# bacchus-snu/bacchus-gpu-controller

Measured on AMD Instinct MI355X. Metric: reconcile p99 (ms) + admission p50 (ms); CR apply→Ready/sec on 8×MI355X node, higher is better.
Workload: dtype none

## Files before the change

native/apiserver/fieldset.cc:

```cpp
#include "apiserver/fieldset.h"

#include "core/json_patch.h"

namespace bgc::apiserver {

using json::Value;

namespace {

enum class ListKind { Atomic, KeyedByUid, Set };

ListKind list_kind(const std::string& path) {
  if (path == "/metadata/ownerReferences") return ListKind::KeyedByUid;
  if (path == "/metadata/finalizers") return ListKind::Set;
  return ListKind::Atomic;
}

bool ignored(const std::string& path, bool include_status) {
  static const std::set<std::string> kIgnored = {
      "/apiVersion", "/kind", "/metadata/name", "/metadata/namespace", "/metadata/resourceVersion",
      "/metadata/uid", "/metadata/generation", "/metadata/creationTimestamp", "/metadata/managedFields",
      "/metadata/selfLink", "/metadata/deletionTimestamp", "/metadata/deletionGracePeriodSeconds"};
  if (kIgnored.count(path)) return true;
  if (!include_status && (path == "/status" || path.rfind("/status/", 0) == 0)) return true;
  return false;
}

void collect(const Value& v, const std::string& path, FieldSet& out, bool include_status) {
  if (!path.empty() && ignored(path, include_status)) return;
  if (v.is_object() && !v.empty()) {
    const auto& keys = v.keys();
    const auto& vals = v.values();
    for (size_t i = 0; i < keys.size(); ++i) {
      collect(vals[i], path + "/" + json::escape_pointer_token(keys[i]), out, include_status);
    }
    return;
  }
  if (v.is_array() && !v.empty()) {
    ListKind lk = list_kind(path);
    if (lk == ListKind::KeyedByUid) {
      for (const auto& item : v.items()) {
        out.insert(path + "/[uid=" + json::escape_pointer_token(item.get_string("uid")) + "]");
      }
      return;
    }
    if (lk == ListKind::Set) {
      for (const auto& item : v.items()) out.insert(path + "/[=" + json::escape_pointer_token(item.dump()) + "]");
      return;
    }
  }
  if (!path.empty()) out.insert(path);
}

class Tokens {
 public:
  explicit Tokens(std::string_view p) : p_(p), i_(p.empty() ? 1 : 1), end_(p.empty()) {}
  bool next(std::string_view& tok) {
    if (end_ || i_ > p_.size()) return false;
    size_t j = p_.find('/', i_);
    std::string_view raw = p_.substr(i_, j == std::string_view::npos ? std::string_view::npos : j - i_);
    if (j == std::string_view::npos) end_ = true;
    else i_ = j + 1;
    if (raw.find('~') == std::string_view::npos) {
      tok = raw;
      return true;
    }
    scratch_.clear();
    for (size_t k = 0; k < raw.size(); ++k) {
      if (raw[k] == '~' && k + 1 < raw.size()) {
        scratch_.push_back(raw[k + 1] == '1' ? '/' : '~');
        ++k;
      } else {
        scratch_.push_back(raw[k]);
      }
    }
    tok = scratch_;
    return true;
  }
  bool last() const { return end_; }

 private:
  std::string_view p_;
  size_t i_;
  bool end_;
  std::string scratch_;
};

bool is_item_token(std::string_view t) { return t.size() >= 3 && t.front() == '[' && t.back() == ']'; }

long find_item(const Value& arr, std::string_view tok) {
  std::string_view inner = tok.substr(1, tok.size() - 2);
  if (inner.substr(0, 4) == "uid=") {
    std::string_view uid = inner.substr(4);
    for (size_t i = 0; i < arr.size(); ++i) {
      const Value& u = arr[i].get("uid");
      if (u.is_string() && u.as_string() == uid) return static_cast<long>(i);
    }
    return -1;
  }
  if (!inner.empty() && inner.front() == '=') {
    Value want;
    if (!json::try_parse(inner.substr(1), want, nullptr)) return -1;
    for (size_t i = 0; i < arr.size(); ++i) {
      if (arr[i] == want) return static_cast<long>(i);
    }
  }
  return -1;
}

}

FieldSet leaves(const Value& obj, bool include_status) {
  FieldSet fs;
  collect(obj, "", fs, include_status);
  return fs;
}

const Value* get_path(const Value& root, const std::string& path) {
  const Value* cur = &root;
  Tokens ts(path);
  std::string_view t;
  while (ts.next(t)) {
    if (is_item_token(t)) {
      if (!cur->is_array()) return nullptr;
      long i = find_item(*cur, t);
      if (i < 0) return nullptr;
      cur = &(*cur)[static_cast<size_t>(i)];
    } else {
      cur = cur->find(t);
      if (!cur) return nullptr;
    }
  }
  return cur;
}

bool remove_path(Value& root, const std::string& path) {
  Value* cur = &root;
  Tokens ts(path);
  std::string_view t;
  while (ts.next(t)) {
    const bool last = ts.last();
    if (is_item_token(t)) {
      if (!cur->is_array()) return false;
      long i = find_item(*cur, t);
      if (i < 0) return false;
      if (last) {
        cur->erase_index(static_cast<size_t>(i));
        return true;
      }
      cur = &(*cur)[static_cast<size_t>(i)];
    } else {
      if (last) return cur->erase(t);
      cur = cur->find_mut(t);
      if (!cur) return false;
    }
  }
  return false;
}

void set_path(Value& root, const std::string& path, const Value& v) {
  Value* cur = &root;
  Tokens ts(path);
  std::string_view t;
  while (ts.next(t)) {
    const bool last = ts.last();
    if (is_item_token(t)) {
      if (!cur->is_array()) *cur = Value::array();
      long i = find_item(*cur, t);
      if (i < 0) {
        cur->push_back(last ? v : Value::object());
        cur = &(*cur)[cur->size() - 1];
      } else {
        cur = &(*cur)[static_cast<size_t>(i)];
        if (last) *cur = v;
      }
      continue;
    }
    if (!cur->is_object()) *cur = Value::object();
    if (last) {
      (*cur)[t] = v;
    } else {
      cur = &(*cur)[t];
    }
  }
}

void diff_leaves(const Value& before, const Value& after, FieldSet& changed, FieldSet& removed, bool include_status) {
  FieldSet b = leaves(before, include_status);
  FieldSet a = leaves(after, include_status);
  for (const auto& p : a) {
    const Value* bv = b.count(p) ? get_path(before, p) : nullptr;
    const Value* av = get_path(after, p);
    if (!bv || !av || !(*bv == *av)) changed.insert(p);
  }
  for (const auto& p : b) {
    if (!a.count(p)) removed.insert(p);
  }
}

void diff_member_leaves(const Value& before, const Value& after, const std::string& key, FieldSet& changed,
                        FieldSet& removed) {
  const std::string base = "/" + json::escape_pointer_token(key);
  FieldSet b, a;
  if (const Value* v = before.find(key)) collect(*v, base, b, true);
  if (const Value* v = after.find(key)) collect(*v, base, a, true);
  for (const auto& p : a) {
    const Value* bv = b.count(p) ? get_path(before, p) : nullptr;
    const Value* av = get_path(after, p);
    if (!bv || !av || !(*bv == *av)) changed.insert(p);
  }
  for (const auto& p : b) {
    if (!a.count(p)) removed.insert(p);
  }
}

std::string display_path(const std::string& path) {
  std::string out;
  Tokens ts(path);
  std::string_view t;
  while (ts.next(t)) {
    if (!is_item_token(t)) out += '.';
    out.append(t.data(), t.size());
  }
  return out;
}

Value fields_v1(const FieldSet& fs) {
  Value root = Value::object();
  for (const auto& p : fs) {
    Value* cur = &root;
    Tokens ts(p);
    std::string_view t;
    std::string key;
    while (ts.next(t)) {
      key.clear();
      if (is_item_token(t)) {
        std::string_view inner = t.substr(1, t.size() - 2);
        if (inner.substr(0, 4) == "uid=") key = "k:{\"uid\":" + json::quote(std::string(inner.substr(4))) + "}";
        else key.append("v:").append(inner.substr(1));
      } else {
        key.append("f:").append(t);
      }
      cur = &(*cur)[key];
      if (cur->is_null()) *cur = Value::object();
    }
  }
  return root;
}

}
```

native/apiserver/fieldset.h:

```cpp
#pragma once

#include <map>
#include <set>
#include <string>
#include <vector>

#include "core/json.h"

namespace bgc::apiserver {

using FieldSet = std::set<std::string>;

FieldSet leaves(const json::Value& obj, bool include_status = false);
const json::Value* get_path(const json::Value& root, const std::string& path);
bool remove_path(json::Value& root, const std::string& path);
void set_path(json::Value& root, const std::string& path, const json::Value& v);
void diff_leaves(const json::Value& before, const json::Value& after, FieldSet& changed, FieldSet& removed,
                 bool include_status = false);
void diff_member_leaves(const json::Value& before, const json::Value& after, const std::string& key,
                        FieldSet& changed, FieldSet& removed);
std::string display_path(const std::string& path);
json::Value fields_v1(const FieldSet& fs);

}
```

native/apiserver/server.cc:

```cpp
#include "apiserver/server.h"

#include <algorithm>
#include <array>
#include <atomic>
#include <chrono>
#include <condition_variable>
#include <deque>
#include <functional>
#include <iterator>
#include <mutex>
#include <optional>
#include <regex>
#include <set>
#include <sstream>
#include <thread>
#include <unordered_map>
#include <unordered_set>

#include <openssl/crypto.h>

#include "apiserver/fieldset.h"
#include "core/crypto.h"
#include "core/http.h"
#include "core/json_patch.h"
#include "core/log.h"
#include "core/metrics.h"
#include "core/process.h"
#include "core/stall.h"
#include "core/trace.h"
#include "core/net.h"
#include "core/yaml.h"
#include "crd/schema.h"
#include "kube/leader.h"
#include "kube/quantity.h"
#include "kube/resource.h"

namespace bgc::apiserver {

using json::Value;
using kube::ResourceType;

namespace {


struct StatusError : std::runtime_error {
  int code;
  std::string reason;
  Value details;
  StatusError(int c, std::string r, const std::string& msg, Value d = {})
      : std::runtime_error(msg), code(c), reason(std::move(r)), details(std::move(d)) {}
};

Value status_body(int code, const std::string& reason, const std::string& message, const Value& details = {}) {
  Value s = Value::object({{"kind", "Status"}, {"apiVersion", "v1"}, {"metadata", Value::object()},
                           {"status", code < 400 ? "Success" : "Failure"}, {"message", message},
                           {"reason", reason}});
  if (!details.is_null()) s["details"] = details;
  s["code"] = code;
  return s;
}

std::string resource_ref(const ResourceType& rt) {
  return rt.group.empty() ? rt.plural : rt.plural + "." + rt.group;
}

StatusError not_found(const ResourceType& rt, const std::string& name) {
  return StatusError(404, "NotFound", resource_ref(rt) + " \"" + name + "\" not found",
                     Value::object({{"name", name}, {"group", rt.group}, {"kind", rt.plural}}));
}

StatusError already_exists(const ResourceType& rt, const std::string& name) {
  return StatusError(409, "AlreadyExists", resource_ref(rt) + " \"" + name + "\" already exists",
                     Value::object({{"name", name}, {"group", rt.group}, {"kind", rt.plural}}));
}

StatusError conflict(const ResourceType& rt, const std::string& name) {
  return StatusError(409, "Conflict",
                     "Operation cannot be fulfilled on " + resource_ref(rt) + " \"" + name +
                         "\": the object has been modified; please apply your changes to the latest version and try again",
                     Value::object({{"name", name}, {"group", rt.group}, {"kind", rt.plural}}));
}

StatusError invalid(const ResourceType& rt, const std::string& name, const std::string& msg) {
  return StatusError(422, "Invalid", rt.kind + "." + rt.group + " \"" + name + "\" is invalid: " + msg,
                     Value::object({{"name", name}, {"group", rt.group}, {"kind", rt.kind}}));
}

std::string now_rfc3339() {
  std::string s = kube::rfc3339_micro_now();
  return s.substr(0, 19) + "Z";
}

bool dns1123_label(const std::string& s) {
  if (s.empty() || s.size() > 63) return false;
  for (size_t i = 0; i < s.size(); ++i) {
    char c = s[i];
    bool ok = (c >= 'a' && c <= 'z') || (c >= '0' && c <= '9') || (c == '-' && i != 0 && i + 1 != s.size());
    if (!ok) return false;
  }
  return true;
}

bool dns1123_subdomain(const std::string& s) {
  if (s.empty() || s.size() > 253) return false;
  size_t start = 0;
  while (true) {
    size_t dot = s.find('.', start);
    std::string part = s.substr(start, dot == std::string::npos ? std::string::npos : dot - start);
    if (!dns1123_label(part)) return false;
    if (dot == std::string::npos) return true;
    start = dot + 1;
  }
}


struct Requirement {
  std::string key;
  std::string op;
  std::vector<std::string> values;
};

std::string trim(std::string s) {
  while (!s.empty() && s.front() == ' ') s.erase(0, 1);
  while (!s.empty() && s.back() == ' ') s.pop_back();
  return s;
}

std::vector<Requirement> parse_selector(const std::string& sel) {
  std::vector<Requirement> out;
  std::vector<std::string> parts;
  int depth = 0;
  std::string cur;
  for (char c : sel) {
    if (c == '(') ++depth;
    if (c == ')') --depth;
    if (c == ',' && depth == 0) {
      parts.push_back(cur);
      cur.clear();
    } else {
      cur.push_back(c);
    }
  }
  if (!cur.empty()) parts.push_back(cur);
  for (auto p : parts) {
    p = trim(p);
    if (p.empty()) continue;
    Requirement r;
    size_t pos;
    if (p[0] == '!') {
      r.key = trim(p.substr(1));
      r.op = "!exists";
    } else if ((pos = p.find(" notin ")) != std::string::npos || (pos = p.find(" in ")) != std::string::npos) {
      bool notin = p.compare(pos, 7, " notin ") == 0;
      r.key = trim(p.substr(0, pos));
      r.op = notin ? "notin" : "in";
      size_t lp = p.find('('), rp = p.rfind(')');
      if (lp == std::string::npos || rp == std::string::npos) throw StatusError(400, "BadRequest", "invalid selector: " + p);
      std::string inner = p.substr(lp + 1, rp - lp - 1);
      std::stringstream ss(inner);
      std::string v;
      while (std::getline(ss, v, ',')) r.values.push_back(trim(v));
    } else if ((pos = p.find("!=")) != std::string::npos) {
      r.key = trim(p.substr(0, pos));
      r.op = "!=";
      r.values.push_back(trim(p.substr(pos + 2)));
    } else if ((pos = p.find("==")) != std::string::npos) {
      r.key = trim(p.substr(0, pos));
      r.op = "=";
      r.values.push_back(trim(p.substr(pos + 2)));
    } else if ((pos = p.find('=')) != std::string::npos) {
      r.key = trim(p.substr(0, pos));
      r.op = "=";
      r.values.push_back(trim(p.substr(pos + 1)));
    } else {
      r.key = p;
      r.op = "exists";
    }
    out.push_back(r);
  }
  return out;
}

bool selector_matches(const std::vector<Requirement>& reqs, const Value& obj) {
  const Value& labels = obj.get("metadata").get("labels");
  for (const auto& r : reqs) {
    const Value* v = labels.find(r.key);
    bool has = v && v->is_string();
    std::string val = has ? v->as_string() : "";
    if (r.op == "exists" && !has) return false;
    if (r.op == "!exists" && has) return false;
    if (r.op == "=" && (!has || val != r.values[0])) return false;
    if (r.op == "!=" && has && val == r.values[0]) return false;
    if (r.op == "in" && (!has || std::find(r.values.begin(), r.values.end(), val) == r.values.end())) return false;
    if (r.op == "notin" && has && std::find(r.values.begin(), r.values.end(), val) != r.values.end()) return false;
  }
  return true;
}

struct FieldFilter {
  std::string name, ns;
  std::string name_prefix;
  bool name_ok(std::string_view n) const {
    return (name.empty() || n == name) && (name_prefix.empty() || n.substr(0, name_prefix.size()) == name_prefix);
  }
};

FieldFilter parse_field_selector(const std::string& s) {
  FieldFilter f;
  std::stringstream ss(s);
  std::string part;
  while (std::getline(ss, part, ',')) {
    size_t eq = part.find('=');
    if (eq == std::string::npos) continue;
    std::string k = trim(part.substr(0, eq));
    std::string v = trim(part.substr(part[eq + 1] == '=' ? eq + 2 : eq + 1));
    if (k == "metadata.name") f.name = v;
    else if (k == "metadata.namespace") f.ns = v;
    else if (k == "kube-lite.test/name-prefix") f.name_prefix = v;
  }
  return f;
}


struct UserInfo {
  std::string username;
  std::string uid;
  std::vector<std::string> groups;
  bool is_admin() const { return std::find(groups.begin(), groups.end(), "system:masters") != groups.end(); }
  Value to_json() const {
    Value g = Value::array();
    for (auto& x : groups) g.push_back(x);
    Value v = Value::object({{"username", username}});
    if (!uid.empty()) v["uid"] = uid;
    v["groups"] = g;
    return v;
  }
};

struct TypeStore;

struct TypeInfo {
  ResourceType rt;
  std::shared_ptr<const Value> schema;
  bool custom = false;
  std::shared_ptr<TypeStore> store;
  std::string key() const { return rt.group + "/" + rt.version + "/" + rt.plural; }
};

struct ManagerEntry {
  std::string operation;
  std::string api_version;
  std::string time;
  std::string subresource;
  FieldSet fields;
  bool operator==(const ManagerEntry& o) const {
    return operation == o.operation && fields == o.fields && subresource == o.subresource;
  }
};
using Managers = std::map<std::string, ManagerEntry>;

inline const std::shared_ptr<const Managers>& no_managers() {
  static const std::shared_ptr<const Managers> empty = std::make_shared<const Managers>();
  return empty;
}

struct Stored {
  std::shared_ptr<const Value> obj;
  uint64_t rv = 0;
  std::weak_ptr<const std::string> line;
  std::shared_ptr<const Managers> managers = no_managers();
};

bool wants_metadata(const http::Request& req) {
  const std::string* a = req.headers.get("Accept");
  return a && a->find("as=PartialObjectMetadata") != std::string::npos;
}

void dump_partial_metadata(const Value& obj, std::string& out) {
  out += "{\"kind\":\"PartialObjectMetadata\",\"apiVersion\":\"meta.k8s.io/v1\",\"metadata\":";
  obj.get("metadata").dump_to(out);
  out += "}";
}

std::string partial_metadata_line(const std::string& line) {
  std::string_view body(line);
  while (!body.empty() && (body.back() == '\n' || body.back() == '\r')) body.remove_suffix(1);
  const std::string_view type = json::raw_member(body, "type");
  const std::string_view md = json::raw_member(json::raw_member(body, "object"), "metadata");
  std::string out;
  out.reserve(md.size() + 128);
  out += "{\"type\":";
  out.append(type.data(), type.size());
  out += ",\"object\":{\"kind\":\"PartialObjectMetadata\",\"apiVersion\":\"meta.k8s.io/v1\",\"metadata\":";
  if (md.empty()) out += "{}";
  else out.append(md.data(), md.size());
  out += "}}\n";
  return out;
}

enum class View : uint8_t { AsIs, Added, Deleted };

struct EventRec {
  uint64_t rv;
  std::string type_key;
  std::string ns;
  std::shared_ptr<const Value> meta;
  std::shared_ptr<const std::string> line;
  struct Transitions {
    std::shared_ptr<const Value> prev_meta;
    std::shared_ptr<const std::string> prev_line;
    std::once_flag added_once, deleted_once;
    std::string added, added_meta, deleted, deleted_meta;
  };
  std::unique_ptr<Transitions> tr;
  const std::string& metadata_line() const {
    std::call_once(meta_once_, [this] { meta_line_ = partial_metadata_line(*line); });
    return meta_line_;
  }
  const std::string& line_as(View v, bool meta_only) const {
    if (v == View::AsIs || !tr) return meta_only ? metadata_line() : *line;
    Transitions& t = *tr;
    if (v == View::Added) {
      std::call_once(t.added_once, [&] {
        t.added = retyped_line(*line, "ADDED");
        t.added_meta = partial_metadata_line(t.added);
      });
      return meta_only ? t.added_meta : t.added;
    }
    std::call_once(t.deleted_once, [&] {
      t.deleted = deleted_from_prev();
      t.deleted_meta = partial_metadata_line(t.deleted);
    });
    return meta_only ? t.deleted_meta : t.deleted;
  }

 private:
  static std::string retyped_line(const std::string& l, const char* type) {
    const std::string_view t = json::raw_member(l, "type");
    std::string out;
    if (t.empty()) return l;
    out.reserve(l.size() + 8);
    out.append(l, 0, static_cast<size_t>(t.data() - l.data()));
    out += '"';
    out += type;
    out += '"';
    out.append(t.data() + t.size(), l.data() + l.size());
    return out;
  }
  std::string deleted_from_prev() const {
    std::string_view prev(*tr->prev_line);
    while (!prev.empty() && (prev.back() == '\n' || prev.back() == '\r')) prev.remove_suffix(1);
    const std::string_view obj = json::raw_member(prev, "object");
    const std::string_view old_rv = json::raw_member(json::raw_member(obj, "metadata"), "resourceVersion");
    const std::string_view new_rv =
        json::raw_member(json::raw_member(json::raw_member(*line, "object"), "metadata"), "resourceVersion");
    std::string out = "{\"type\":\"DELETED\",\"object\":";
    if (old_rv.empty()) {
      out.append(obj.data(), obj.size());
    } else {
      out.append(obj.data(), static_cast<size_t>(old_rv.data() - obj.data()));
      out.append(new_rv.data(), new_rv.size());
      out.append(old_rv.data() + old_rv.size(), obj.data() + obj.size());
    }
    out += "}\n";
    return out;
  }
  mutable std::once_flag meta_once_;
  mutable std::string meta_line_;
};

struct QueuedEvent {
  std::shared_ptr<const EventRec> e;
  View view = View::AsIs;
};

std::shared_ptr<const Value> filter_view(const Value& obj) {
  const Value& m = obj.get("metadata");
  Value meta = Value::object({{"name", m.get("name")}});
  if (m.contains("labels")) meta["labels"] = m.get("labels");
  return std::make_shared<const Value>(Value::object({{"metadata", std::move(meta)}}));
}

struct WatchSub {
  std::string type_key;
  std::string ns;
  std::vector<Requirement> sel;
  FieldFilter fields;
  std::mutex m;
  std::condition_variable cv;
  std::deque<QueuedEvent> q;
  bool closed = false;
  bool overflow = false;

  void close() {
    {
      std::lock_guard<std::mutex> g(m);
      closed = true;
    }
    cv.notify_one();
  }
};

class RwLock {
 public:
  RwLock() {
    const char* kind = std::getenv("BGC_KL_RWLOCK");
    mutex_only_ = !kind || (std::string(kind) != "writer" && std::string(kind) != "reader");
    pthread_rwlockattr_t a;
    pthread_rwlockattr_init(&a);
    pthread_rwlockattr_setkind_np(&a, kind && std::string(kind) == "reader" ? PTHREAD_RWLOCK_PREFER_READER_NP
                                                                           : PTHREAD_RWLOCK_PREFER_WRITER_NONRECURSIVE_NP);
    pthread_rwlock_init(&l_, &a);
    pthread_rwlockattr_destroy(&a);
  }
  ~RwLock() { pthread_rwlock_destroy(&l_); }
  RwLock(const RwLock&) = delete;
  RwLock& operator=(const RwLock&) = delete;
  void lock() {
    if (mutex_only_) m_.lock();
    else pthread_rwlock_wrlock(&l_);
  }
  bool try_lock() { return mutex_only_ ? m_.try_lock() : pthread_rwlock_trywrlock(&l_) == 0; }
  void unlock() {
    if (mutex_only_) m_.unlock();
    else pthread_rwlock_unlock(&l_);
  }
  void lock_shared() {
    if (mutex_only_) m_.lock();
    else pthread_rwlock_rdlock(&l_);
  }
  bool try_lock_shared() { return mutex_only_ ? m_.try_lock() : pthread_rwlock_tryrdlock(&l_) == 0; }
  void unlock_shared() { unlock(); }

 private:
  pthread_rwlock_t l_;
  std::mutex m_;
  bool mutex_only_ = false;
};

thread_local std::vector<std::shared_ptr<WatchSub>> t_pending_wakeups;
thread_local std::vector<std::shared_ptr<const EventRec>> t_retired_events;

inline void flush_watch_wakeups() {
  for (auto& w : t_pending_wakeups) w->cv.notify_one();
  t_pending_wakeups.clear();
  t_retired_events.clear();
}

struct LockStats {
  std::atomic<uint64_t> acquisitions{0}, shared{0}, contended{0}, wait_ns{0}, hold_ns{0};
};

class StoreLock {
 public:
  StoreLock(RwLock& m, LockStats& st, LockStats* also = nullptr) : m_(m), st_(st), also_(also) {
    if (!m_.try_lock()) {
      int64_t t0 = metrics::now_ns();
      m_.lock();
      const auto waited = static_cast<uint64_t>(metrics::now_ns() - t0);
      st_.contended.fetch_add(1, std::memory_order_relaxed);
      st_.wait_ns.fetch_add(waited, std::memory_order_relaxed);
      if (also_) {
        also_->contended.fetch_add(1, std::memory_order_relaxed);
        also_->wait_ns.fetch_add(waited, std::memory_order_relaxed);
      }
    }
    t_acq_ = metrics::now_ns();
  }
  ~StoreLock() {
    const auto held = static_cast<uint64_t>(metrics::now_ns() - t_acq_);
    st_.acquisitions.fetch_add(1, std::memory_order_relaxed);
    st_.hold_ns.fetch_add(held, std::memory_order_relaxed);
    if (also_) {
      also_->acquisitions.fetch_add(1, std::memory_order_relaxed);
      also_->hold_ns.fetch_add(held, std::memory_order_relaxed);
    }
    m_.unlock();
    flush_watch_wakeups();
  }
  StoreLock(const StoreLock&) = delete;
  StoreLock& operator=(const StoreLock&) = delete;

 private:
  RwLock& m_;
  LockStats& st_;
  LockStats* also_;
  int64_t t_acq_ = 0;
};

class SharedStoreLock {
 public:
  SharedStoreLock(RwLock& m, LockStats& st) : m_(m) {
    if (!m_.try_lock_shared()) {
      int64_t t0 = metrics::now_ns();
      m_.lock_shared();
      st.contended.fetch_add(1, std::memory_order_relaxed);
      st.wait_ns.fetch_add(static_cast<uint64_t>(metrics::now_ns() - t0), std::memory_order_relaxed);
    }
    st.shared.fetch_add(1, std::memory_order_relaxed);
  }
  ~SharedStoreLock() { m_.unlock_shared(); }
  SharedStoreLock(const SharedStoreLock&) = delete;
  SharedStoreLock& operator=(const SharedStoreLock&) = delete;

 private:
  RwLock& m_;
};

struct TypeStore {
  struct Shard {
    RwLock mu;
    std::unordered_map<std::string, Stored> objs;
  };
  class Shards {
   public:
    explicit Shards(size_t n) : n_(std::max<size_t>(1, n)), p_(new Shard[n_]) {}
    Shard* begin() { return p_.get(); }
    Shard* end() { return p_.get() + n_; }
    std::reverse_iterator<Shard*> rbegin() { return std::reverse_iterator<Shard*>(end()); }
    std::reverse_iterator<Shard*> rend() { return std::reverse_iterator<Shard*>(begin()); }
    size_t size() const { return n_; }
    Shard& operator[](size_t i) { return p_[i]; }

   private:
    size_t n_;
    std::unique_ptr<Shard[]> p_;
  };
  explicit TypeStore(size_t n_shards) : shards(n_shards) {}
  Shards shards;
  Shard& shard(const std::string& key) {
    return shards.size() == 1 ? shards[0] : shards[std::hash<std::string>{}(key) % shards.size()];
  }
  RwLock seq;
  std::atomic<uint64_t> version{0};
  LockStats stats;
  LockStats seq_stats;
  std::deque<std::shared_ptr<const EventRec>> history;
  uint64_t compacted_rv = 0;
  std::mutex watches_mu;
  std::set<std::shared_ptr<WatchSub>> watches;
};

class AllShards {
 public:
  AllShards(TypeStore& ts, bool exclusive) : ts_(ts), exclusive_(exclusive) {
    for (auto& sh : ts_.shards) {
      if (exclusive_) {
        if (!sh.mu.try_lock()) {
          const int64_t t0 = metrics::now_ns();
          sh.mu.lock();
          ts_.stats.contended.fetch_add(1, std::memory_order_relaxed);
          ts_.stats.wait_ns.fetch_add(static_cast<uint64_t>(metrics::now_ns() - t0), std::memory_order_relaxed);
        }
      } else if (!sh.mu.try_lock_shared()) {
        const int64_t t0 = metrics::now_ns();
        sh.mu.lock_shared();
        ts_.stats.contended.fetch_add(1, std::memory_order_relaxed);
        ts_.stats.wait_ns.fetch_add(static_cast<uint64_t>(metrics::now_ns() - t0), std::memory_order_relaxed);
      }
    }
    ts_.stats.acquisitions.fetch_add(1, std::memory_order_relaxed);
  }
  ~AllShards() {
    for (auto it = ts_.shards.rbegin(); it != ts_.shards.rend(); ++it) {
      if (exclusive_) it->mu.unlock();
      else it->mu.unlock_shared();
    }
    flush_watch_wakeups();
  }
  AllShards(const AllShards&) = delete;
  AllShards& operator=(const AllShards&) = delete;

 private:
  TypeStore& ts_;
  bool exclusive_;
};

struct FaultRule {
  std::string method;
  std::regex path;
  std::string path_src;
  int status = 0;
  int retry_after_s = -1;
  int delay_ms = 0;
  int hold_ms = 0;
  int remaining = -1;
  bool reset = false;
  std::string message;
};

struct ParsedPath {
  TypeInfo* ti = nullptr;
  std::string ns;
  std::string name;
  std::string sub;
  bool collection = false;
};

thread_local std::string t_trace_tag;
thread_local std::string t_trace_name;

void trace_step(const std::string& name, const char* step) {
  if (!t_trace_tag.empty()) trace::mark(name, t_trace_tag + step);
}

struct WriteResult {
  std::shared_ptr<const Value> obj;
  int code = 200;
  std::shared_ptr<const std::string> line;
  std::string_view body() const {
    static const std::string kPrefixEnd = ",\"object\":";
    if (!line) return {};
    size_t at = line->find(kPrefixEnd);
    if (at == std::string::npos || line->size() < at + kPrefixEnd.size() + 2) return {};
    at += kPrefixEnd.size();
    return std::string_view(*line).substr(at, line->size() - at - 2);
  }
};

std::string obj_key(const ResourceType& rt, const std::string& ns, const std::string& name) { return rt.key(ns, name); }

}


struct ApiServer::Impl {
  Options opts;
  std::unique_ptr<http::Server> server;

  RwLock types_mu;
  std::map<std::string, TypeInfo> types;
  std::atomic<uint64_t> rv{1000};
  std::mutex index_mu;
  std::unordered_map<std::string, std::pair<std::string, std::string>> by_uid;
  using Ref = std::pair<std::string, std::string>;
  struct RefHash {
    size_t operator()(const Ref& r) const { return std::hash<std::string>{}(r.first) * 31 + std::hash<std::string>{}(r.second); }
  };
  std::unordered_map<std::string, std::unordered_set<Ref, RefHash>> by_owner;
  std::unordered_map<std::string, std::unordered_set<Ref, RefHash>> by_namespace;

  struct GcItem {
    bool is_namespace = false;
    std::string id;
    bool finish_namespace = false;
  };
  std::mutex gc_mu;
  std::condition_variable gc_cv;
  std::deque<GcItem> gc_queue;
  bool gc_stop = false;
  std::atomic<uint64_t> gc_collected{0};
  std::vector<std::thread> gc_threads;

  std::unordered_map<std::string, UserInfo> tokens;

  std::mutex fault_mu;
  std::vector<FaultRule> faults;

  struct ListSnapshot {
    uint64_t rv = 0;
    std::vector<std::shared_ptr<const Value>> items;
    std::chrono::steady_clock::time_point expires;
  };
  std::mutex list_mu;
  std::map<uint64_t, ListSnapshot> list_snapshots;
  uint64_t next_list_id = 1;
  std::atomic<uint64_t> list_pages{0};

  static constexpr uint64_t kRvMask = 0x5bd1e9955bd1e995ULL;
  std::string rv_str(uint64_t v) const {
    if (!opts.opaque_rv) return std::to_string(v);
    static const char* digits = "0123456789abcdefghijklmnopqrstuvwxyz";
    uint64_t x = v ^ kRvMask;
    std::string out;
    do {
      out.insert(out.begin(), digits[x % 36]);
      x /= 36;
    } while (x);
    return "kl." + out;
  }
  bool parse_rv(const std::string& s, uint64_t* v) const {
    if (!opts.opaque_rv) {
      if (s.empty() || s.find_first_not_of("0123456789") != std::string::npos) return false;
      *v = std::strtoull(s.c_str(), nullptr, 10);
      return true;
    }
    if (s.rfind("kl.", 0) != 0 || s.size() < 4) return false;
    uint64_t x = 0;
    for (size_t i = 3; i < s.size(); ++i) {
      const char c = s[i];
      int d = c >= '0' && c <= '9' ? c - '0' : c >= 'a' && c <= 'z' ? c - 'a' + 10 : -1;
      if (d < 0) return false;
      x = x * 36 + static_cast<uint64_t>(d);
    }
    *v = x ^ kRvMask;
    return true;
  }

  std::mutex hook_mu;
  struct FastHook {
    std::shared_ptr<const Value> cfg;
    std::shared_ptr<http::Client> client;
    std::string path;
  };
  std::map<const Value*, FastHook> hook_fast;
  std::map<std::string, std::shared_ptr<http::Client>> hook_clients;
  std::atomic<bool> webhook_h2{false};
  std::atomic<int64_t> write_latency_us{0};
  std::atomic<int> watch_coalesce_us{0};

  std::atomic<uint64_t> requests{0};
  std::atomic<uint64_t> faults_hit{0};
  LockStats types_stats;

  explicit Impl(Options o) : opts(std::move(o)) {
    if (const char* e = std::getenv("BGC_KL_STORE_SHARDS"); e && *e) opts.store_shards = std::max(1, std::atoi(e));
    watch_coalesce_us = opts.watch_coalesce_us;
    if (const char* e = std::getenv("BGC_KL_H2_CALLER_READS"); e && *e) opts.webhook_h2_caller_reads = std::string(e) != "0";
    webhook_h2 = opts.webhook_http2;
    write_latency_us = opts.write_latency_us;
    for (const ResourceType* rt : kube::types::builtin()) {
      TypeInfo ti;
      ti.rt = *rt;
      ti.store = std::make_shared<TypeStore>(opts.store_shards);
      types[ti.key()] = ti;
    }
    if (!opts.token_file.empty()) load_tokens(opts.token_file);
    const TypeInfo& ns_ti = types.at(kube::types::Namespace.group + "/" + kube::types::Namespace.version + "/" +
                                     kube::types::Namespace.plural);
    for (const char* name : {"default", "kube-system", "kube-public", "kube-node-lease"}) {
      const uint64_t v = ++rv;
      Value ns = Value::object(
          {{"apiVersion", "v1"}, {"kind", "Namespace"},
           {"metadata", Value::object({{"name", name}, {"uid", crypto::uuid_v4()}, {"creationTimestamp", now_rfc3339()},
                                       {"resourceVersion", rv_str(v)}})},
           {"spec", Value::object({{"finalizers", Value::array({Value("kubernetes")})}})},
           {"status", Value::object({{"phase", "Active"}})}});
      Stored st;
      st.obj = std::make_shared<const Value>(std::move(ns));
      st.rv = v;
      ns_ti.store->shard(obj_key(ns_ti.rt, "", name)).objs[obj_key(ns_ti.rt, "", name)] = std::move(st);
    }
    for (int i = 0; i < std::max(1, opts.gc_workers); ++i) gc_threads.emplace_back([this] {
      gc_loop();
      OPENSSL_thread_stop();
    });
  }

  ~Impl() {
    {
      std::lock_guard<std::mutex> g(gc_mu);
      gc_stop = true;
    }
    gc_cv.notify_all();
    for (auto& t : gc_threads) t.join();
  }

  template <typename F>
  void for_each_store(F f) {
    std::vector<std::pair<std::string, std::shared_ptr<TypeStore>>> stores;
    {
      SharedStoreLock lk(types_mu, types_stats);
      for (auto& [k, ti] : types) stores.emplace_back(k, ti.store);
    }
    for (auto& [k, st] : stores) f(k, *st);
  }

  TypeInfo* type_by_key(const std::string& key) {
    SharedStoreLock lk(types_mu, types_stats);
    auto it = types.find(key);
    return it == types.end() ? nullptr : &it->second;
  }

  void load_tokens(const std::string& path) {
    std::stringstream ss(net::read_file(path));
    std::string line;
    while (std::getline(ss, line)) {
      if (line.empty() || line[0] == '#') continue;
      std::vector<std::string> cols;
      std::string cur;
      bool q = false;
      for (char c : line) {
        if (c == '"') {
          q = !q;
          continue;
        }
        if (c == ',' && !q) {
          cols.push_back(cur);
          cur.clear();
          continue;
        }
        cur.push_back(c);
      }
      cols.push_back(cur);
      if (cols.size() < 2) continue;
      UserInfo u;
      u.username = cols[1];
      if (cols.size() > 2) u.uid = cols[2];
      if (cols.size() > 3 && !cols[3].empty()) {
        std::stringstream gs(cols[3]);
        std::string g;
        while (std::getline(gs, g, ',')) u.groups.push_back(g);
      }
      u.groups.push_back("system:authenticated");
      tokens[cols[0]] = u;
    }
  }

  UserInfo authenticate(const http::Request& req) {
    UserInfo u;
    std::string auth = req.headers.get_or("Authorization");
    if (auth.rfind("Bearer ", 0) == 0) {
      auto it = tokens.find(auth.substr(7));
      if (it == tokens.end()) throw StatusError(401, "Unauthorized", "Unauthorized");
      u = it->second;
    } else if (!req.peer_cn.empty()) {
      u.username = req.peer_cn;
      u.groups = req.peer_orgs;
      u.groups.push_back("system:authenticated");
    } else if (opts.anonymous_admin) {
      u.username = "system:admin";
      u.groups = {"system:masters", "system:authenticated"};
    } else {
      throw StatusError(401, "Unauthorized", "Unauthorized");
    }
    if (const std::string* imp = req.headers.get("Impersonate-User")) {
      if (!u.is_admin()) {
        throw StatusError(403, "Forbidden", "users \"" + *imp + "\" is forbidden: User \"" + u.username +
                                                "\" cannot impersonate resource \"users\" in API group \"\" at the cluster scope");
      }
      UserInfo imp_u;
      imp_u.username = *imp;
      for (const auto& kv : req.headers.items()) {
        std::string lk = kv.first;
        for (auto& c : lk) c = static_cast<char>(std::tolower(static_cast<unsigned char>(c)));
        if (lk == "impersonate-group") {
          std::stringstream gs(kv.second);
          std::string g;
          while (std::getline(gs, g, ',')) {
            if (!trim(g).empty()) imp_u.groups.push_back(trim(g));
          }
        }
      }
      imp_u.groups.push_back("system:authenticated");
      u = imp_u;
    }
    return u;
  }

  TypeInfo* find_type(const std::string& group, const std::string& version, const std::string& plural) {
    auto it = types.find(group + "/" + version + "/" + plural);
    return it == types.end() ? nullptr : &it->second;
  }

  bool parse_path(const std::string& path, ParsedPath& out, std::string& group, std::string& version,
                  std::vector<std::string>& rest) {
    std::vector<std::string> segs;
    std::stringstream ss(path);
    std::string s;
    while (std::getline(ss, s, '/')) {
      if (!s.empty()) segs.push_back(s);
    }
    size_t i = 0;
    if (segs.size() >= 2 && segs[0] == "api") {
      group = "";
      version = segs[1];
      i = 2;
    } else if (segs.size() >= 3 && segs[0] == "apis") {
      group = segs[1];
      version = segs[2];
      i = 3;
    } else {
      return false;
    }
    rest.assign(segs.begin() + static_cast<long>(i), segs.end());
    if (rest.empty()) return false;
    SharedStoreLock lk(types_mu, types_stats);
    if (rest[0] == "namespaces" && rest.size() >= 3) {
      TypeInfo* ti = find_type(group, version, rest[2]);
      if (ti && ti->rt.namespaced) {
        out.ti = ti;
        out.ns = rest[1];
        out.collection = rest.size() == 3;
        if (rest.size() >= 4) out.name = rest[3];
        if (rest.size() >= 5) out.sub = rest[4];
        return true;
      }
    }
    TypeInfo* ti = find_type(group, version, rest[0]);
    if (!ti) throw StatusError(404, "NotFound", "the server could not find the requested resource");
    out.ti = ti;
    out.collection = rest.size() == 1;
    if (rest.size() >= 2) out.name = rest[1];
    if (rest.size() >= 3) out.sub = rest[2];
    return true;
  }

  struct PreparedEvent {
    std::string head, tail;
    bool ok = false;
    std::shared_ptr<const Value> filter;
    std::shared_ptr<EventRec> rec;
  };

  std::shared_ptr<const std::string> emit_locked(const TypeInfo& ti, const std::string& ns, uint64_t ev_rv,
                                                 std::string line, std::shared_ptr<const Value> filter,
                                                 std::shared_ptr<EventRec> rec) {
    TypeStore& st = *ti.store;
    st.version.fetch_add(1, std::memory_order_release);
    if (!rec) rec = std::make_shared<EventRec>();
    rec->rv = ev_rv;
    rec->type_key = ti.key();
    rec->ns = ns;
    rec->meta = std::move(filter);
    rec->line = std::make_shared<const std::string>(std::move(line));
    st.history.push_back(rec);
    while (st.history.size() > opts.history_limit) {
      st.compacted_rv = st.history.front()->rv;
      t_retired_events.push_back(std::move(st.history.front()));
      st.history.pop_front();
    }
    const std::string& name = rec->meta->get("metadata").get_string("name");
    std::lock_guard<std::mutex> wg(st.watches_mu);
    for (const auto& w : st.watches) {
      if (!w->ns.empty() && w->ns != ns) continue;
      if (!w->fields.name_ok(name)) continue;
      View view;
      if (!view_for(w->sel, *rec, &view)) continue;
      {
        std::lock_guard<std::mutex> g(w->m);
        if (w->q.size() > 100000) w->overflow = true;
        else w->q.push_back({rec, view});
      }
      t_pending_wakeups.push_back(w);
    }
    return rec->line;
  }

  static bool view_for(const std::vector<Requirement>& sel, const EventRec& e, View* view) {
    *view = View::AsIs;
    if (sel.empty()) return true;
    const bool now_in = selector_matches(sel, *e.meta);
    if (!e.tr) return now_in;
    const bool was_in = selector_matches(sel, *e.tr->prev_meta);
    if (now_in && !was_in) *view = View::Added;
    else if (!now_in && was_in) *view = View::Deleted;
    return now_in || was_in;
  }

  struct HookMatch {
    std::string name;
    std::shared_ptr<const Value> cfg;
    const Value* hook;
  };
  std::mutex hook_match_mu;
  uint64_t hook_match_version = ~uint64_t{0};
  std::unordered_map<std::string, std::vector<HookMatch>> hook_match_cache;

  std::vector<HookMatch> matching_webhooks(const TypeInfo& ti, const std::string& sub, const std::string& op) {
    TypeInfo* mwc = type_by_key(kube::types::MutatingWebhookConfiguration.group + "/v1/mutatingwebhookconfigurations");
    if (!mwc) return {};
    const std::string cache_key = ti.key() + "|" + sub + "|" + op;
    {
      std::lock_guard<std::mutex> g(hook_match_mu);
      if (hook_match_version == mwc->store->version.load(std::memory_order_acquire)) {
        auto it = hook_match_cache.find(cache_key);
        if (it != hook_match_cache.end()) return it->second;
      }
    }
    std::vector<HookMatch> out;
    AllShards lk(*mwc->store, false);
    const uint64_t version = mwc->store->version.load(std::memory_order_acquire);
    std::string res = ti.rt.plural + (sub.empty() ? "" : "/" + sub);
    for (auto& sh : mwc->store->shards)
    for (auto& kv : sh.objs) {
      for (const auto& hook : kv.second.obj->get("webhooks").items()) {
        for (const auto& rule : hook.get("rules").items()) {
          auto contains = [](const Value& arr, const std::string& v) {
            for (const auto& x : arr.items()) {
              if (x.is_string() && (x.as_string() == "*" || x.as_string() == v)) return true;
            }
            return false;
          };
          bool res_ok = false;
          for (const auto& r : rule.get("resources").items()) {
            std::string rs = r.as_string();
            if (rs == res || rs == "*/*" || (rs == "*" && sub.empty()) ||
                (sub.size() && rs == "*/" + sub) || (rs == ti.rt.plural + "/*")) {
              res_ok = true;
            }
          }
          if (contains(rule.get("apiGroups"), ti.rt.group) && contains(rule.get("apiVersions"), ti.rt.version) &&
              contains(rule.get("operations"), op) && res_ok) {
            out.push_back({hook.get_string("name"), kv.second.obj, &hook});
            break;
          }
        }
      }
    }
    {
      std::lock_guard<std::mutex> g(hook_match_mu);
      if (hook_match_version != version) {
        hook_match_cache.clear();
        hook_match_version = version;
      }
      hook_match_cache[cache_key] = out;
    }
    return out;
  }

  std::shared_ptr<http::Client> hook_client(const HookMatch& hm, std::string& path_out) {
    {
      std::lock_guard<std::mutex> lk(hook_mu);
      auto it = hook_fast.find(hm.hook);
      if (it != hook_fast.end()) {
        path_out = it->second.path;
        return it->second.client;
      }
    }
    auto c = hook_client_slow(*hm.hook, path_out);
    std::lock_guard<std::mutex> lk(hook_mu);
    if (hook_fast.size() > 256) hook_fast.clear();
    hook_fast[hm.hook] = {hm.cfg, c, path_out};
    return c;
  }

  std::shared_ptr<http::Client> hook_client_slow(const Value& hook, std::string& path_out) {
    const Value& cc = hook.get("clientConfig");
    std::string ca = cc.get_string("caBundle");
    std::string base, server_name;
    if (cc.get("url").is_string()) {
      http::Url u = http::parse_url(cc.get_string("url"));
      base = u.scheme + "://" + u.host + ":" + std::to_string(u.port);
      path_out = u.path.empty() ? "/" : u.path;
    } else {
      const Value& svc = cc.get("service");
      std::string ns = svc.get_string("namespace"), name = svc.get_string("name");
      int port = svc.get("port").is_int() ? static_cast<int>(svc.get("port").as_int()) : 443;
      path_out = svc.get_string("path", "/");
      server_name = name + "." + ns + ".svc";
      auto ov = opts.service_overrides.find(ns + "/" + name);
      std::string hostport = ov != opts.service_overrides.end() ? ov->second : server_name + ":" + std::to_string(port);
      base = "https://" + hostport;
    }
    std::string key = base + "|" + server_name + "|" + crypto::sha256_hex(ca);
    std::lock_guard<std::mutex> lk(hook_mu);
    auto it = hook_clients.find(key);
    if (it != hook_clients.end()) return it->second;
    http::ClientOptions o;
    o.base_url = base;
    o.tls_server_name = server_name;
    o.http2 = webhook_h2.load();
    o.h2_connections = opts.webhook_h2_connections;
    o.h2_caller_reads = opts.webhook_h2_caller_reads;
    if (base.rfind("https", 0) == 0) {
      o.tls = net::TlsContext::client(ca.empty() ? "" : crypto::base64_decode(ca), false);
    }
    auto c = std::make_shared<http::Client>(o);
    hook_clients[key] = c;
    return c;
  }

  void call_webhooks(const TypeInfo& ti, const std::string& sub, const std::string& op, const std::string& ns,
                     const std::string& name, Value* obj, const Value* old, const UserInfo& user) {
    auto hooks = matching_webhooks(ti, sub, op);
    if (hooks.empty()) return;
    static auto& hist = metrics::Registry::global().histogram("kl_webhook_duration_seconds", "Webhook callout latency");
    static auto& calls = metrics::Registry::global().counter("kl_webhook_calls_total", "Webhook callouts (any outcome)");
    static auto& ring = [] () -> metrics::SampleLog& {
      auto& r = metrics::Registry::global().samples("webhook");
      r.link("kl_webhook_calls_total", &calls);
      return r;
    }();
    for (const auto& hm : hooks) {
      const Value& hook = *hm.hook;
      std::string fail_policy = hook.get_string("failurePolicy", "Fail");
      int timeout_s = hook.get("timeoutSeconds").is_int() ? static_cast<int>(hook.get("timeoutSeconds").as_int()) : 10;
      std::string uid = crypto::uuid_v4();
      const std::string opts_kind = op == "CREATE" ? "CreateOptions" : op == "DELETE" ? "DeleteOptions" : "UpdateOptions";
      const std::string gvk = "{\"group\":" + json::quote(ti.rt.group) + ",\"version\":" + json::quote(ti.rt.version) +
                              ",\"kind\":" + json::quote(ti.rt.kind) + "}";
      const std::string gvr = "{\"group\":" + json::quote(ti.rt.group) + ",\"version\":" + json::quote(ti.rt.version) +
                              ",\"resource\":" + json::quote(ti.rt.plural) + "}";
      std::string body;
      body.reserve(1024 + (obj ? 2048 : 0) + (old ? 2048 : 0));
      body += "{\"kind\":\"AdmissionReview\",\"apiVersion\":\"admission.k8s.io/v1\",\"request\":{\"uid\":";
      body += json::quote(uid);
      body += ",\"kind\":" + gvk + ",\"resource\":" + gvr;
      if (!sub.empty()) body += ",\"subResource\":" + json::quote(sub);
      body += ",\"requestKind\":" + gvk + ",\"requestResource\":" + gvr;
      if (!sub.empty()) body += ",\"requestSubResource\":" + json::quote(sub);
      body += ",\"name\":" + json::quote(name);
      if (!ns.empty()) body += ",\"namespace\":" + json::quote(ns);
      body += ",\"operation\":" + json::quote(op);
      body += ",\"userInfo\":";
      user.to_json().dump_to(body);
      body += ",\"object\":";
      if (obj) obj->dump_to(body);
      else body += "null";
      body += ",\"oldObject\":";
      if (old) old->dump_to(body);
      else body += "null";
      body += ",\"dryRun\":false,\"options\":{\"kind\":" + json::quote(opts_kind) +
              ",\"apiVersion\":\"meta.k8s.io/v1\"}}}";
      std::string err;
      Value resp_review;
      int64_t t0 = metrics::now_ns();
      try {
        std::string path;
        auto client = hook_client(hm, path);
        http::Headers h;
        h.set("Content-Type", "application/json");
        h.set("Accept", "application/json");
        http::Response r = client->request("POST", path + "?timeout=" + std::to_string(timeout_s) + "s",
                                           body, &h, timeout_s * 1000);
        if (r.status != 200) {
          err = "expected webhook response status code 200, got " + std::to_string(r.status) + ": " + r.body;
        } else if (!json::try_parse(r.body, resp_review, &err)) {
          err = "failed to parse webhook response: " + err;
        }
      } catch (const std::exception& e) {
        err = e.what();
      }
      double secs = static_cast<double>(metrics::now_ns() - t0) * 1e-9;
      hist.observe(secs);
      ring.add(secs, &calls);
      const Value& resp = resp_review.get("response");
      if (err.empty() && !resp.is_object()) err = "webhook response was absent";
      if (err.empty() && resp.get_string("uid") != uid) {
        err = "expected response.uid=\"" + uid + "\", got \"" + resp.get_string("uid") + "\"";
      }
      if (!err.empty()) {
        if (fail_policy == "Ignore") {
          LOG_WARN("apiserver") << "failed calling webhook " << hm.name << " (ignored): " << err;
          continue;
        }
        throw StatusError(500, "InternalError",
                          "Internal error occurred: failed calling webhook \"" + hm.name + "\": " + err);
      }
      if (!resp.get("allowed").is_bool() || !resp.get("allowed").as_bool()) {
        const Value& st = resp.get("status");
        int code = st.get("code").is_int() ? static_cast<int>(st.get("code").as_int()) : 0;
        if (code < 400) code = 400;
        std::string reason = st.get_string("reason", code == 403 ? "Forbidden" : "BadRequest");
        std::string msg = "admission webhook \"" + hm.name + "\" denied the request";
        std::string m = st.get_string("message");
        msg += m.empty() ? " without explanation" : ": " + m;
        throw StatusError(code, reason, msg);
      }
      if (resp.get("patch").is_string() && obj) {
        if (resp.get_string("patchType", "JSONPatch") != "JSONPatch") {
          throw StatusError(500, "InternalError", "unsupported patchType from webhook " + hm.name);
        }
        Value patch;
        std::string perr;
        if (!json::try_parse(crypto::base64_decode(resp.get_string("patch")), patch, &perr)) {
          throw StatusError(500, "InternalError", "invalid patch from webhook " + hm.name + ": " + perr);
        }
        try {
          json::apply_patch(*obj, patch);
        } catch (const std::exception& e) {
          throw StatusError(500, "InternalError",
                            "Internal error occurred: failed calling webhook \"" + hm.name + "\": " + e.what());
        }
      }
    }
  }

  void validate_object(const TypeInfo& ti, const std::string& name, const std::string& ns, const Value& obj) {
    const Value& meta = obj.get("metadata");
    if (ti.rt.plural == "namespaces") {
      if (!dns1123_label(name)) {
        throw invalid(ti.rt, name, "metadata.name: Invalid value: \"" + name +
                                       "\": a lowercase RFC 1123 label must consist of lower case alphanumeric characters or '-', and must start and end with an alphanumeric character");
      }
    } else if (!dns1123_subdomain(name)) {
      throw invalid(ti.rt, name, "metadata.name: Invalid value: \"" + name +
                                     "\": a lowercase RFC 1123 subdomain must consist of lower case alphanumeric characters, '-' or '.', and must start and end with an alphanumeric character");
    }
    if (meta.get("namespace").is_string() && ti.rt.namespaced && meta.get_string("namespace") != ns) {
      throw StatusError(400, "BadRequest", "the namespace of the provided object does not match the namespace sent on the request");
    }
    for (const auto& ref : meta.get("ownerReferences").items()) {
      for (const char* f : {"apiVersion", "kind", "name", "uid"}) {
        if (!ref.get(f).is_string() || ref.get_string(f).empty()) {
          throw invalid(ti.rt, name, std::string("metadata.ownerReferences.") + f + ": Invalid value: \"\": " + f +
                                         " must not be empty");
        }
      }
    }
    if (ti.rt.plural == "rolebindings" || ti.rt.plural == "clusterrolebindings") {
      if (!obj.get("roleRef").is_object()) throw invalid(ti.rt, name, "roleRef: Required value");
    }
    std::shared_ptr<const Value> schema = std::atomic_load(&ti.schema);
    if (opts.validate_schema && ti.custom && schema && schema->is_object()) {
      auto errs = crd::validate(obj, *schema);
      if (!errs.empty()) {
        std::string msg;
        for (size_t i = 0; i < errs.size() && i < 5; ++i) {
          if (i) msg += ", ";
          const auto& e = errs[i];
          if (e.kind == "required") msg += e.path + ": Required value";
          else msg += e.path + ": Invalid value: " + e.detail;
        }
        throw invalid(ti.rt, name, msg);
      }
    }
  }

  void register_crd(const Value& crd) {
    const Value& spec = crd.get("spec");
    std::string group = spec.get_string("group");
    const Value& names = spec.get("names");
    bool namespaced = spec.get_string("scope") == "Namespaced";
    StoreLock lk(types_mu, types_stats);
    for (const auto& v : spec.get("versions").items()) {
      if (v.get("served").is_bool() && !v.get("served").as_bool()) continue;
      TypeInfo ti;
      ti.rt.group = group;
      ti.rt.version = v.get_string("name");
      ti.rt.kind = names.get_string("kind");
      ti.rt.plural = names.get_string("plural");
      ti.rt.namespaced = namespaced;
      ti.rt.has_status = v.get("subresources").get("status").is_object();
      auto schema = std::make_shared<const Value>(v.get("schema").get("openAPIV3Schema"));
      ti.custom = true;
      auto it = types.find(ti.key());
      if (it != types.end()) {
        std::atomic_store(&it->second.schema, schema);
        continue;
      }
      ti.schema = schema;
      ti.store = std::make_shared<TypeStore>(opts.store_shards);
      types[ti.key()] = ti;
    }
  }

  enum class NsPhase { Missing, Active, Terminating };
  NsPhase namespace_phase(const std::string& ns) {
    TypeInfo* nti = type_by_key(kube::types::Namespace.group + "/v1/namespaces");
    if (!nti) return NsPhase::Missing;
    const std::string key = obj_key(nti->rt, "", ns);
    auto& sh = nti->store->shard(key);
    SharedStoreLock lk(sh.mu, nti->store->stats);
    auto it = sh.objs.find(key);
    if (it == sh.objs.end()) return NsPhase::Missing;
    if (!it->second.obj->get("metadata").contains("deletionTimestamp")) return NsPhase::Active;
    return opts.namespace_termination ? NsPhase::Terminating : NsPhase::Missing;
  }

  static bool is_core_namespaces(const TypeInfo& ti) { return ti.rt.plural == "namespaces" && ti.rt.group.empty(); }

  std::shared_ptr<const Value> terminate_namespace_locked(const TypeInfo& ti, const std::string& name, Stored& cur) {
    Value obj = *cur.obj;
    obj["metadata"]["deletionTimestamp"] = now_rfc3339();
    obj["metadata"]["deletionGracePeriodSeconds"] = 0;
    obj["status"]["phase"] = "Terminating";
    auto ptr = commit_locked(ti, "", name, std::move(obj), *cur.managers, &cur);
    std::lock_guard<std::mutex> g(gc_mu);
    gc_queue.push_back({true, name, true});
    gc_cv.notify_one();
    return ptr;
  }

  void finish_namespace(const std::string& name) {
    TypeInfo* nti = type_by_key(kube::types::Namespace.group + "/v1/namespaces");
    if (!nti) return;
    const std::string key = obj_key(nti->rt, "", name);
    auto& sh = nti->store->shard(key);
    StoreLock lk(sh.mu, nti->store->stats);
    auto it = sh.objs.find(key);
    if (it == sh.objs.end() || !it->second.obj->get("metadata").contains("deletionTimestamp")) return;
    if (it->second.obj->get("metadata").get("finalizers").empty()) {
      erase_locked(*nti, "", name);
      return;
    }
    Value obj = *it->second.obj;
    if (obj.get("spec").get("finalizers").empty()) return;
    obj["spec"]["finalizers"] = Value::array();
    commit_locked(*nti, "", name, std::move(obj), *it->second.managers, &it->second);
  }

  static void render_managed(Value& obj, const Managers& m, const std::string& api_version) {
    Value arr = Value::array();
    for (const auto& [key, e] : m) {
      if (e.fields.empty()) continue;
      std::string mgr = key.substr(0, key.find('\x1f'));
      Value ent = Value::object({{"manager", mgr}, {"operation", e.operation},
                                 {"apiVersion", e.api_version.empty() ? api_version : e.api_version},
                                 {"time", e.time}, {"fieldsType", "FieldsV1"}, {"fieldsV1", fields_v1(e.fields)}});
      if (!e.subresource.empty()) ent["subresource"] = e.subresource;
      arr.push_back(std::move(ent));
    }
    if (arr.empty()) obj["metadata"].erase("managedFields");
    else obj["metadata"]["managedFields"] = std::move(arr);
  }

  static bool same_content(const Value& a, const Value& b) {
    if (!a.is_object() || !b.is_object()) return a == b;
    auto volatile_key = [](const std::string& k) { return k == "managedFields" || k == "resourceVersion"; };
    auto count = [&](const Value& v, bool meta) {
      size_t n = 0;
      for (const auto& k : v.keys()) n += (meta && volatile_key(k)) ? 0 : 1;
      return n;
    };
    if (a.size() != b.size()) return false;
    for (size_t i = 0; i < a.keys().size(); ++i) {
      const std::string& k = a.keys()[i];
      const Value* bv = b.find(k);
      if (!bv) return false;
      const Value& av = a.values()[i];
      if (k != "metadata") {
        if (!(av == *bv)) return false;
        continue;
      }
      if (!av.is_object() || !bv->is_object()) {
        if (!(av == *bv)) return false;
        continue;
      }
      if (count(av, true) != count(*bv, true)) return false;
      for (size_t j = 0; j < av.keys().size(); ++j) {
        const std::string& mk = av.keys()[j];
        if (volatile_key(mk)) continue;
        const Value* bm = bv->find(mk);
        if (!bm || !(av.values()[j] == *bm)) return false;
      }
    }
    return true;
  }

  static bool spec_changed(const Value& a, const Value& b) {
    if (!a.is_object() || !b.is_object()) return !(a == b);
    auto skip = [](const std::string& k) { return k == "metadata" || k == "status"; };
    size_t na = 0, nb = 0;
    for (size_t i = 0; i < a.keys().size(); ++i) {
      const std::string& k = a.keys()[i];
      if (skip(k)) continue;
      ++na;
      const Value* bv = b.find(k);
      if (!bv || !(a.values()[i] == *bv)) return true;
    }
    for (const auto& k : b.keys()) nb += skip(k) ? 0 : 1;
    return na != nb;
  }

  static void attribute_update(Managers& m, const std::string& manager, const Value& before, const Value& after,
                               bool status_write, const std::string& api_version) {
    FieldSet changed, removed;
    if (status_write) diff_member_leaves(before, after, "status", changed, removed);
    else diff_leaves(before, after, changed, removed);
    for (auto& [name, e] : m) {
      for (const auto& p : changed) e.fields.erase(p);
      for (const auto& p : removed) e.fields.erase(p);
    }
    if (!changed.empty()) {
      auto& e = m[status_write ? manager + "\x1fstatus" : manager];
      if (e.operation.empty()) {
        e.operation = "Update";
        e.api_version = api_version;
      }
      if (e.operation == "Apply") {
        e.operation = "Update";
      }
      e.time = now_rfc3339();
      if (status_write) e.subresource = "status";
      for (const auto& p : changed) e.fields.insert(p);
    }
    for (auto it = m.begin(); it != m.end();) {
      if (it->second.fields.empty()) it = m.erase(it);
      else ++it;
    }
  }

  static const std::string& rv_placeholder() {
    static const std::string p = "\x01rv\x01";
    return p;
  }
  static PreparedEvent prepare_commit(Value& obj, const Managers& managers, const std::string& api_version,
                                      const char* type) {
    obj["metadata"]["resourceVersion"] = rv_placeholder();
    render_managed(obj, managers, api_version);
    std::string line = std::string("{\"type\":\"") + type + "\",\"object\":";
    obj.dump_to(line);
    line += "}\n";
    static const std::string needle = "\"resourceVersion\":" + Value(rv_placeholder()).dump();
    PreparedEvent pe;
    pe.filter = filter_view(obj);
    pe.rec = std::make_shared<EventRec>();
    size_t pos = line.find(needle);
    if (pos == std::string::npos) return pe;
    pe.head.assign(line, 0, pos);
    pe.head += "\"resourceVersion\":\"";
    pe.tail.assign(line, pos + needle.size() - 1, std::string::npos);
    pe.ok = true;
    return pe;
  }

  std::shared_ptr<const Value> commit_locked(const TypeInfo& ti, const std::string& ns, const std::string& name,
                                            Value obj, Managers managers, const Stored* prev,
                                            const PreparedEvent* pe = nullptr, bool* dangling = nullptr,
                                            std::shared_ptr<const std::string>* line_out = nullptr) {
    TypeStore& ts = *ti.store;
    PreparedEvent local;
    if (!pe || !pe->ok) {
      local = prepare_commit(obj, managers, ti.rt.api_version(), prev ? "MODIFIED" : "ADDED");
      pe = &local;
    }
    std::string key = obj_key(ti.rt, ns, name);
    Ref ref{ti.key(), key};
    {
      std::lock_guard<std::mutex> ig(index_mu);
      if (prev) unindex_owners_locked(*prev->obj, ref);
      by_uid[obj.get("metadata").get_string("uid")] = ref;
      const Value& owners = obj.get("metadata").get("ownerReferences");
      for (const auto& r : owners.items()) by_owner[r.get_string("uid")].insert(ref);
      if (ti.rt.namespaced) by_namespace[ns].insert(ref);
      if (dangling && !prev && !owners.empty()) {
        bool alive = false;
        for (const auto& r : owners.items()) alive = alive || by_uid.count(r.get_string("uid")) > 0;
        *dangling = !alive;
      }
    }
    std::shared_ptr<EventRec> rec = pe->rec ? pe->rec : std::make_shared<EventRec>();
    if (prev && opts.selector_transitions &&
        prev->obj->get("metadata").get("labels") != obj.get("metadata").get("labels")) {
      auto t = std::make_unique<EventRec::Transitions>();
      t->prev_meta = filter_view(*prev->obj);
      if (auto held = prev->line.lock()) {
        t->prev_line = std::move(held);
      } else {
        std::string l = "{\"type\":\"MODIFIED\",\"object\":";
        prev->obj->dump_to(l);
        l += "}\n";
        t->prev_line = std::make_shared<const std::string>(std::move(l));
      }
      rec->tr = std::move(t);
    }
    uint64_t new_rv;
    std::string digits;
    std::shared_ptr<const std::string> line;
    {
      StoreLock sl(ts.seq, ts.seq_stats);
      new_rv = ++rv;
      digits = rv_str(new_rv);
      std::string preline;
      if (pe->ok) {
        preline.reserve(pe->head.size() + digits.size() + pe->tail.size());
        preline += pe->head;
        preline += digits;
        preline += pe->tail;
      } else {
        obj["metadata"]["resourceVersion"] = digits;
        preline = std::string("{\"type\":\"") + (prev ? "MODIFIED" : "ADDED") + "\",\"object\":";
        obj.dump_to(preline);
        preline += "}\n";
      }
      line = emit_locked(ti, ns, new_rv, std::move(preline), pe->filter ? pe->filter : filter_view(obj), std::move(rec));
    }
    obj["metadata"]["resourceVersion"] = digits;
    auto ptr = std::make_shared<const Value>(std::move(obj));
    Stored s;
    s.obj = ptr;
    s.rv = new_rv;
    s.managers = std::make_shared<const Managers>(std::move(managers));
    s.line = line;
    ts.shard(key).objs[key] = std::move(s);
    if (line_out) *line_out = std::move(line);
    return ptr;
  }

  void unindex_owners_locked(const Value& obj, const Ref& ref) {
    for (const auto& r : obj.get("metadata").get("ownerReferences").items()) {
      auto it = by_owner.find(r.get_string("uid"));
      if (it == by_owner.end()) continue;
      it->second.erase(ref);
      if (it->second.empty()) by_owner.erase(it);
    }
  }

  void erase_locked(const TypeInfo& ti, const std::string& ns, const std::string& name) {
    TypeStore& ts = *ti.store;
    std::string key = obj_key(ti.rt, ns, name);
    auto& b = ts.shard(key).objs;
    auto it = b.find(key);
    if (it == b.end()) return;
    std::shared_ptr<const Value> ptr = it->second.obj;
    std::string line = "{\"type\":\"DELETED\",\"object\":";
    const size_t obj_at = line.size();
    static const std::string kObjectKey = ",\"object\":";
    const std::shared_ptr<const std::string> held = it->second.line.lock();
    const std::string* committed = held.get();
    const size_t at = committed ? committed->find(kObjectKey) : std::string::npos;
    if (at != std::string::npos && committed->size() >= at + kObjectKey.size() + 2) {
      line.append(*committed, at + kObjectKey.size(), committed->size() - (at + kObjectKey.size()) - 2);
    } else {
      ptr->dump_to(line);
    }
    line += "}\n";
    const std::string old_rv = "\"resourceVersion\":" + json::quote(ptr->get("metadata").get_string("resourceVersion"));
    const size_t pos = line.find(old_rv, obj_at);
    auto filter = filter_view(*ptr);
    std::string uid = ptr->get("metadata").get_string("uid");
    Ref ref{ti.key(), key};
    bool has_dependents;
    {
      std::lock_guard<std::mutex> ig(index_mu);
      by_uid.erase(uid);
      unindex_owners_locked(*ptr, ref);
      if (ti.rt.namespaced) {
        auto nit = by_namespace.find(ns);
        if (nit != by_namespace.end()) {
          nit->second.erase(ref);
          if (nit->second.empty()) by_namespace.erase(nit);
        }
      }
      has_dependents = by_owner.count(uid) > 0;
    }
    uint64_t new_rv;
    {
      StoreLock sl(ts.seq, ts.seq_stats);
      new_rv = ++rv;
      const std::string digits = rv_str(new_rv);
      if (pos != std::string::npos) {
        line.replace(pos, old_rv.size(), "\"resourceVersion\":\"" + digits + "\"");
      } else {
        Value final_obj = *ptr;
        final_obj["metadata"]["resourceVersion"] = digits;
        line = "{\"type\":\"DELETED\",\"object\":";
        final_obj.dump_to(line);
        line += "}\n";
      }
      emit_locked(ti, ns, new_rv, std::move(line), std::move(filter), nullptr);
    }
    b.erase(it);
    bool is_ns = ti.rt.plural == "namespaces" && ti.rt.group.empty();
    if (has_dependents || is_ns) {
      std::lock_guard<std::mutex> g(gc_mu);
      if (has_dependents) gc_queue.push_back({false, uid});
      if (is_ns) gc_queue.push_back({true, name});
      gc_cv.notify_one();
    }
  }

  void gc_loop() {
    while (true) {
      GcItem item;
      {
        std::unique_lock<std::mutex> g(gc_mu);
        gc_cv.wait(g, [&] { return gc_stop || !gc_queue.empty(); });
        if (gc_stop) return;
        item = std::move(gc_queue.front());
        gc_queue.pop_front();
      }
      std::vector<Ref> victims;
      {
        std::lock_guard<std::mutex> ig(index_mu);
        auto& idx = item.is_namespace ? by_namespace : by_owner;
        auto it = idx.find(item.id);
        if (it != idx.end()) victims.assign(it->second.begin(), it->second.end());
      }
      for (const auto& v : victims) {
        TypeInfo* vti = type_by_key(v.first);
        if (!vti) continue;
        auto& vsh = vti->store->shard(v.second);
        StoreLock lk(vsh.mu, vti->store->stats);
        auto it = vsh.objs.find(v.second);
        if (it == vsh.objs.end()) continue;
        const Value& meta = it->second.obj->get("metadata");
        if (!item.is_namespace) {
          bool alive = false;
          {
            std::lock_guard<std::mutex> ig(index_mu);
            for (const auto& r : meta.get("ownerReferences").items()) alive = alive || by_uid.count(r.get_string("uid")) > 0;
          }
          if (alive) continue;
        }
        std::string vns = meta.get_string("namespace"), vname = meta.get_string("name");
        if (is_core_namespaces(*vti) && opts.namespace_termination) {
          if (!meta.contains("deletionTimestamp")) terminate_namespace_locked(*vti, vname, it->second);
          continue;
        }
        erase_locked(*vti, vns, vname);
        gc_collected.fetch_add(1, std::memory_order_relaxed);
      }
      if (item.finish_namespace) finish_namespace(item.id);
    }
  }

  static void canonicalize_quantities(const TypeInfo& ti, Value& obj) {
    if (ti.custom || (ti.rt.plural != "resourcequotas" && ti.rt.plural != "nodes")) return;
    auto fix = [](Value* m) {
      if (!m || !m->is_object()) return;
      for (Value& v : m->items_mut()) {
        std::string text;
        if (v.is_string()) text = v.as_string();
        else if (v.is_int()) text = v.dump();
        else continue;
        if (auto c = kube::canonical_quantity(text)) {
          if (!v.is_string() || *c != text) v = Value(std::move(*c));
        }
      }
    };
    auto sub = [](Value& o, const char* k) { return o.is_object() ? o.find_mut(k) : nullptr; };
    Value* spec = sub(obj, "spec");
    Value* status = sub(obj, "status");
    if (ti.rt.plural == "resourcequotas") {
      if (spec) fix(sub(*spec, "hard"));
      if (status) {
        fix(sub(*status, "hard"));
        fix(sub(*status, "used"));
      }
    } else if (status) {
      fix(sub(*status, "capacity"));
      fix(sub(*status, "allocatable"));
    }
  }

  using Compute = std::function<std::pair<Value, Managers>(const Stored* cur)>;

  WriteResult write(TypeInfo& ti, const std::string& ns, const std::string& name, const std::string& sub,
                    const UserInfo& user, const Compute& compute, bool allow_create, bool is_status) {
    for (int attempt = 0; attempt < 8; ++attempt) {
      Stored cur_copy;
      bool exists = false;
      const std::string key = obj_key(ti.rt, ns, name);
      auto& sh = ti.store->shard(key);
      {
        SharedStoreLock lk(sh.mu, ti.store->stats);
        auto it = sh.objs.find(key);
        if (it != sh.objs.end()) {
          cur_copy = it->second;
          exists = true;
        }
      }
      if (!exists && !allow_create) throw not_found(ti.rt, name);
      auto [obj, managers] = compute(exists ? &cur_copy : nullptr);
      canonicalize_quantities(ti, obj);
      std::string op = exists ? "UPDATE" : "CREATE";
      if (!exists && ti.rt.namespaced) {
        const NsPhase phase = namespace_phase(ns);
        if (phase == NsPhase::Missing) {
          throw StatusError(404, "NotFound", "namespaces \"" + ns + "\" not found",
                            Value::object({{"name", ns}, {"kind", "namespaces"}}));
        }
        if (phase == NsPhase::Terminating) {
          throw StatusError(
              403, "Forbidden",
              ti.rt.plural + " \"" + name + "\" is forbidden: unable to create new content in namespace " + ns +
                  " because it is being terminated",
              Value::object({{"name", name}, {"kind", ti.rt.plural},
                             {"causes", Value::array({Value::object({{"reason", "NamespaceTerminating"},
                                                                     {"message", "namespace " + ns + " is being terminated"},
                                                                     {"field", "metadata.namespace"}})})}}));
        }
      }
      if (exists && same_content(obj, *cur_copy.obj) && managers == *cur_copy.managers) {
        return {cur_copy.obj, 200, nullptr};
      }
      trace_step(name, ".hook0");
      call_webhooks(ti, sub, op, ns, name, &obj, exists ? cur_copy.obj.get() : nullptr, user);
      trace_step(name, ".hook1");
      obj["metadata"]["name"] = name;
      if (ti.rt.namespaced) obj["metadata"]["namespace"] = ns;
      else obj["metadata"].erase("namespace");
      canonicalize_quantities(ti, obj);
      validate_object(ti, name, ns, obj);
      if (exists && same_content(obj, *cur_copy.obj) && managers == *cur_copy.managers) {
        return {cur_copy.obj, 200, nullptr};
      }
      if (exists && spec_changed(*cur_copy.obj, obj)) {
        int64_t gen = cur_copy.obj->get("metadata").get("generation").is_int()
                          ? cur_copy.obj->get("metadata").get("generation").as_int()
                          : 1;
        obj["metadata"]["generation"] = gen + 1;
      }
      PreparedEvent pe = prepare_commit(obj, managers, ti.rt.api_version(), exists ? "MODIFIED" : "ADDED");
      StoreLock lk(sh.mu, ti.store->stats);
      auto it = sh.objs.find(key);
      bool now_exists = it != sh.objs.end();
      if (now_exists != exists || (exists && it->second.rv != cur_copy.rv)) continue;
      if (exists) {
        if (obj.get("metadata").contains("deletionTimestamp") && obj.get("metadata").get("finalizers").empty() &&
            !(is_core_namespaces(ti) && opts.namespace_termination && !obj.get("spec").get("finalizers").empty())) {
          erase_locked(ti, ns, name);
          return {cur_copy.obj, 200, nullptr};
        }
        (void)is_status;
        WriteResult wr;
        trace_step(name, ".commit");
        wr.obj = commit_locked(ti, ns, name, std::move(obj), std::move(managers), &it->second, &pe, nullptr, &wr.line);
        return wr;
      }
      if (ti.rt.plural == "customresourcedefinitions") register_crd(obj);
      bool dangling = false;
      std::shared_ptr<const std::string> line;
      trace_step(name, ".commit");
      auto created = commit_locked(ti, ns, name, std::move(obj), std::move(managers), nullptr, &pe, &dangling, &line);
      if (dangling) erase_locked(ti, ns, name);
      WriteResult wr;
      wr.obj = created;
      wr.code = 201;
      wr.line = std::move(line);
      return wr;
    }
    throw conflict(ti.rt, name);
  }

  void init_new(const TypeInfo& ti, Value& obj, const std::string& ns, const std::string& name) {
    obj["apiVersion"] = ti.rt.api_version();
    obj["kind"] = ti.rt.kind;
    Value& meta = obj["metadata"];
    meta["name"] = name;
    if (ti.rt.namespaced) meta["namespace"] = ns;
    meta["uid"] = crypto::uuid_v4();
    meta["creationTimestamp"] = now_rfc3339();
    meta["generation"] = 1;
    meta.erase("resourceVersion");
    meta.erase("deletionTimestamp");
    meta.erase("managedFields");
    if (ti.rt.has_status && ti.custom) obj.erase("status");
    if (ti.rt.plural == "namespaces" && ti.rt.group.empty()) {
      obj["spec"] = Value::object({{"finalizers", Value::array({"kubernetes"})}});
      obj["status"] = Value::object({{"phase", "Active"}});
    }
  }

  static void carry_meta(Value& obj, const Value& cur) {
    const Value& cm = cur.get("metadata");
    Value& m = obj["metadata"];
    for (const char* f : {"uid", "creationTimestamp", "generation", "deletionTimestamp"}) {
      if (cm.contains(f)) m[f] = cm.get(f);
      else m.erase(f);
    }
    obj["apiVersion"] = cur.get("apiVersion");
    obj["kind"] = cur.get("kind");
  }

  std::string field_manager(const http::Request& req, const std::string& dflt) {
    std::string fm = req.query_param("fieldManager");
    if (!fm.empty()) return fm;
    std::string ua = req.headers.get_or("User-Agent", dflt);
    size_t slash = ua.find('/');
    return slash == std::string::npos ? ua : ua.substr(0, slash);
  }

  Value parse_body(const http::Request& req) {
    Value v;
    std::string err;
    std::string ct = req.headers.get_or("Content-Type");
    if (ct.find("yaml") != std::string::npos && !req.body.empty() && req.body[0] != '{') {
      try {
        return yaml::parse(req.body);
      } catch (const std::exception& e) {
        throw StatusError(400, "BadRequest", std::string("error decoding YAML: ") + e.what());
      }
    }
    if (!json::try_parse(req.body, v, &err)) throw StatusError(400, "BadRequest", "couldn't get version/kind; json parse error: " + err);
    return v;
  }

  void do_create(ParsedPath& p, const http::Request& req, const UserInfo& user, http::ResponseWriter& w) {
    Value body = parse_body(req);
    if (!body.is_object()) throw StatusError(400, "BadRequest", "object must be a JSON object");
    std::string name = body.get("metadata").get_string("name");
    if (name.empty()) {
      std::string gen = body.get("metadata").get_string("generateName");
      if (gen.empty()) throw invalid(p.ti->rt, "", "metadata.name: Required value: name or generateName is required");
      static const char* alnum = "bcdfghjklmnpqrstvwxz2456789";
      std::string rnd = crypto::random_bytes(5);
      name = gen;
      for (unsigned char c : rnd) name.push_back(alnum[c % 27]);
    }
    std::string manager = field_manager(req, "unknown");
    if (!t_trace_tag.empty()) t_trace_name = name;
    auto res = write(*p.ti, p.ns, name, "", user,
                     [&](const Stored* cur) -> std::pair<Value, Managers> {
                       if (cur) throw already_exists(p.ti->rt, name);
                       Value obj = body;
                       init_new(*p.ti, obj, p.ns, name);
                       Managers m;
                       attribute_update(m, manager, Value::object(), obj, false, p.ti->rt.api_version());
                       return {std::move(obj), std::move(m)};
                     },
                     true, false);
    {
      std::string_view b = res.body();
      if (!b.empty()) w.send_json(res.code, b);
      else w.send_json(res.code, res.obj->dump());
    }
  }

  void do_update(ParsedPath& p, const http::Request& req, const UserInfo& user, http::ResponseWriter& w) {
    Value body = parse_body(req);
    if (!body.is_object()) throw StatusError(400, "BadRequest", "object must be a JSON object");
    std::string bname = body.get("metadata").get_string("name");
    if (!bname.empty() && bname != p.name) {
      throw StatusError(400, "BadRequest", "the name of the object (" + bname +
                                               ") does not match the name on the URL (" + p.name + ")");
    }
    bool is_status = p.sub == "status";
    std::string manager = field_manager(req, "unknown");
    auto res = write(*p.ti, p.ns, p.name, p.sub, user,
                     [&](const Stored* cur) -> std::pair<Value, Managers> {
                       std::string want_rv = body.get("metadata").get_string("resourceVersion");
                       if (!want_rv.empty() && want_rv != cur->obj->get("metadata").get_string("resourceVersion")) {
                         throw conflict(p.ti->rt, p.name);
                       }
                       Value obj;
                       if (is_status) {
                         obj = *cur->obj;
                         if (body.contains("status")) obj["status"] = body.get("status");
                         else obj.erase("status");
                       } else {
                         obj = body;
                         carry_meta(obj, *cur->obj);
                         if (p.ti->rt.has_status) {
                           if (cur->obj->contains("status")) obj["status"] = cur->obj->get("status");
                           else obj.erase("status");
                         }
                       }
                       Managers m = *cur->managers;
                       attribute_update(m, manager, *cur->obj, obj, is_status, p.ti->rt.api_version());
                       return {std::move(obj), std::move(m)};
                     },
                     false, is_status);
    {
      std::string_view b = res.body();
      if (!b.empty()) w.send_json(res.code, b);
      else w.send_json(res.code, res.obj->dump());
    }
  }

  std::pair<Value, Managers> apply_ssa(const TypeInfo& ti, const Stored* cur, const Value& config,
                                       const std::string& manager_name, bool force, bool is_status,
                                       const std::string& ns, const std::string& name) {
    const std::string manager = is_status ? manager_name + "\x1fstatus" : manager_name;
    FieldSet cfg_fields = leaves(config, is_status);
    if (is_status) {
      FieldSet only;
      for (const auto& f : cfg_fields) {
        if (f == "/status" || f.rfind("/status/", 0) == 0) only.insert(f);
      }
      cfg_fields.swap(only);
    }
    Value live;
    Managers m;
    if (cur) {
      live = *cur->obj;
      m = *cur->managers;
    } else {
      live = Value::object();
      init_new(ti, live, ns, name);
    }
    std::vector<std::pair<std::string, std::string>> conflicts;
    for (const auto& f : cfg_fields) {
      const Value* want = get_path(config, f);
      const Value* have = get_path(live, f);
      for (auto& [other, e] : m) {
        if (other == manager || !e.fields.count(f)) continue;
        if (have && want && *have == *want) continue;
        conflicts.emplace_back(other, f);
      }
    }
    if (!conflicts.empty() && !force) {
      std::string msg = "Apply failed with " + std::to_string(conflicts.size()) + " conflict" +
                        (conflicts.size() > 1 ? "s" : "") + ": ";
      for (size_t i = 0; i < conflicts.size(); ++i) {
        if (i) msg += "; ";
        msg += "conflict with \"" + conflicts[i].first.substr(0, conflicts[i].first.find('\x1f')) + "\": " +
               display_path(conflicts[i].second);
      }
      throw StatusError(409, "Conflict", msg);
    }
    if (force) {
      for (const auto& [other, f] : conflicts) m[other].fields.erase(f);
    }
    if (auto it = m.find(manager); it != m.end()) {
      for (const auto& f : it->second.fields) {
        if (cfg_fields.count(f)) continue;
        bool other_owner = false;
        for (auto& [other, e] : m) {
          if (other != manager && e.fields.count(f)) other_owner = true;
        }
        if (!other_owner) remove_path(live, f);
      }
    }
    for (const auto& f : cfg_fields) {
      if (const Value* v = get_path(config, f)) set_path(live, f, *v);
    }
    auto& me = m[manager];
    me.operation = "Apply";
    me.api_version = ti.rt.api_version();
    me.time = now_rfc3339();
    me.subresource = is_status ? "status" : "";
    me.fields = cfg_fields;
    for (auto it = m.begin(); it != m.end();) {
      if (it->second.fields.empty()) it = m.erase(it);
      else ++it;
    }
    if (cur && ti.rt.has_status && !is_status) {
      if (cur->obj->contains("status")) live["status"] = cur->obj->get("status");
    }
    return {std::move(live), std::move(m)};
  }

  void do_patch(ParsedPath& p, const http::Request& req, const UserInfo& user, http::ResponseWriter& w) {
    std::string ct = req.headers.get_or("Content-Type");
    bool is_status = p.sub == "status";
    bool is_apply = ct.find("apply-patch") != std::string::npos;
    std::string manager = field_manager(req, is_apply ? "" : "unknown");
    if (is_apply && req.query_param("fieldManager").empty()) {
      throw StatusError(400, "BadRequest", "PatchOptions.meta.k8s.io \"\" is invalid: fieldManager: Required value: is required for apply patch");
    }
    Value patch = parse_body(req);
    bool force = req.query_param("force") == "true";
    auto res = write(*p.ti, p.ns, p.name, p.sub, user,
                     [&](const Stored* cur) -> std::pair<Value, Managers> {
                       if (is_apply) {
                         std::string pname = patch.get("metadata").get_string("name");
                         if (!pname.empty() && pname != p.name) {
                           throw StatusError(400, "BadRequest", "the name of the object (" + pname +
                                                                    ") does not match the name on the URL (" + p.name + ")");
                         }
                         return apply_ssa(*p.ti, cur, patch, manager, force, is_status, p.ns, p.name);
                       }
                       Value obj = *cur->obj;
                       try {
                         if (ct.find("json-patch") != std::string::npos) {
                           json::apply_patch(obj, patch);
                         } else {
                           json::apply_merge_patch(obj, patch);
                         }
                       } catch (const json::PatchError& e) {
                         throw StatusError(422, "Invalid", std::string("the server rejected our request due to an error in our request: ") + e.what());
                       }
                       std::string want_rv = obj.get("metadata").get_string("resourceVersion");
                       if (!want_rv.empty() && want_rv != cur->obj->get("metadata").get_string("resourceVersion")) {
                         throw conflict(p.ti->rt, p.name);
                       }
                       if (is_status) {
                         Value keep = *cur->obj;
                         if (obj.contains("status")) keep["status"] = obj.get("status");
                         else keep.erase("status");
                         obj = std::move(keep);
                       } else {
                         carry_meta(obj, *cur->obj);
                         if (p.ti->rt.has_status) {
                           if (cur->obj->contains("status")) obj["status"] = cur->obj->get("status");
                           else obj.erase("status");
                         }
                       }
                       Managers m = *cur->managers;
                       attribute_update(m, manager, *cur->obj, obj, is_status, p.ti->rt.api_version());
                       return {std::move(obj), std::move(m)};
                     },
                     is_apply, is_status);
    {
      std::string_view b = res.body();
      if (!b.empty()) w.send_json(res.code, b);
      else w.send_json(res.code, res.obj->dump());
    }
  }

  void do_delete(ParsedPath& p, const http::Request& req, const UserInfo& user, http::ResponseWriter& w) {
    std::shared_ptr<const Value> cur;
    const std::string key = obj_key(p.ti->rt, p.ns, p.name);
    auto& sh = p.ti->store->shard(key);
    {
      SharedStoreLock lk(sh.mu, p.ti->store->stats);
      auto it = sh.objs.find(key);
      if (it == sh.objs.end()) throw not_found(p.ti->rt, p.name);
      cur = it->second.obj;
    }
    trace_step(p.name, ".hook0");
    call_webhooks(*p.ti, "", "DELETE", p.ns, p.name, nullptr, cur.get(), user);
    trace_step(p.name, ".hook1");
    StoreLock lk(sh.mu, p.ti->store->stats);
    auto it = sh.objs.find(key);
    if (it == sh.objs.end()) throw not_found(p.ti->rt, p.name);
    const Value& meta = it->second.obj->get("metadata");
    if (is_core_namespaces(*p.ti) && opts.namespace_termination) {
      auto ptr = meta.contains("deletionTimestamp") ? it->second.obj
                                                    : terminate_namespace_locked(*p.ti, p.name, it->second);
      w.send_json(200, ptr->dump());
      return;
    }
    if (!meta.get("finalizers").empty()) {
      if (!meta.contains("deletionTimestamp")) {
        Value obj = *it->second.obj;
        obj["metadata"]["deletionTimestamp"] = now_rfc3339();
        obj["metadata"]["deletionGracePeriodSeconds"] = 0;
        auto ptr = commit_locked(*p.ti, p.ns, p.name, std::move(obj), *it->second.managers, &it->second);
        w.send_json(202, ptr->dump());
        return;
      }
      w.send_json(202, it->second.obj->dump());
      return;
    }
    erase_locked(*p.ti, p.ns, p.name);
    (void)req;
    w.send_json(200, status_body(200, "", "").dump());
  }

  void do_get(ParsedPath& p, http::ResponseWriter& w, bool meta_only = false) {
    std::shared_ptr<const Value> obj;
    {
      const std::string key = obj_key(p.ti->rt, p.ns, p.name);
      auto& sh = p.ti->store->shard(key);
      SharedStoreLock lk(sh.mu, p.ti->store->stats);
      auto it = sh.objs.find(key);
      if (it == sh.objs.end()) throw not_found(p.ti->rt, p.name);
      obj = it->second.obj;
    }
    if (meta_only) {
      std::string out;
      dump_partial_metadata(*obj, out);
      w.send_json(200, out);
      return;
    }
    w.send_json(200, obj->dump());
  }

  void do_list(ParsedPath& p, const http::Request& req, http::ResponseWriter& w) {
    const int64_t limit = req.has_query_param("limit") ? std::atoll(req.query_param("limit").c_str()) : 0;
    const std::string cont = req.query_param("continue");
    std::vector<std::shared_ptr<const Value>> items;
    uint64_t list_rv = 0;
    size_t offset = 0;
    uint64_t snap_id = 0;
    if (!cont.empty()) {
      const size_t dot = cont.find('.');
      snap_id = std::strtoull(cont.c_str(), nullptr, 10);
      offset = dot == std::string::npos ? 0 : std::strtoull(cont.c_str() + dot + 1, nullptr, 10);
      std::lock_guard<std::mutex> lk(list_mu);
      auto it = list_snapshots.find(snap_id);
      if (it == list_snapshots.end() || std::chrono::steady_clock::now() > it->second.expires) {
        if (it != list_snapshots.end()) list_snapshots.erase(it);
        throw StatusError(410, "Expired",
                          "The provided continue parameter is too old to display a consistent list result. You can "
                          "start a new list without the continue parameter.");
      }
      list_rv = it->second.rv;
      items = it->second.items;
    } else {
      auto sel = parse_selector(req.query_param("labelSelector"));
      auto ff = parse_field_selector(req.query_param("fieldSelector"));
      {
        AllShards lk(*p.ti->store, false);
        list_rv = rv.load();
        for (auto& sh : p.ti->store->shards)
        for (auto& [k, st] : sh.objs) {
          const Value& meta = st.obj->get("metadata");
          if (!p.ns.empty() && meta.get_string("namespace") != p.ns) continue;
          if (!ff.name_ok(meta.get_string("name"))) continue;
          if (!ff.ns.empty() && meta.get_string("namespace") != ff.ns) continue;
          if (!sel.empty() && !selector_matches(sel, *st.obj)) continue;
          items.push_back(st.obj);
        }
      }
      std::sort(items.begin(), items.end(), [](const auto& a, const auto& b) {
        const Value& ma = a->get("metadata");
        const Value& mb = b->get("metadata");
        return std::make_pair(ma.get_string("namespace"), ma.get_string("name")) <
               std::make_pair(mb.get_string("namespace"), mb.get_string("name"));
      });
    }
    size_t end = items.size();
    std::string next;
    if (limit > 0 && offset + static_cast<size_t>(limit) < items.size()) {
      end = offset + static_cast<size_t>(limit);
      std::lock_guard<std::mutex> lk(list_mu);
      if (snap_id == 0) {
        const auto now = std::chrono::steady_clock::now();
        for (auto it = list_snapshots.begin(); it != list_snapshots.end();) {
          it = now > it->second.expires ? list_snapshots.erase(it) : std::next(it);
        }
        snap_id = next_list_id++;
        list_snapshots[snap_id] = ListSnapshot{list_rv, items, now + std::chrono::milliseconds(opts.continue_ttl_ms)};
      }
      next = std::to_string(snap_id) + "." + std::to_string(end);
    } else if (snap_id != 0) {
      std::lock_guard<std::mutex> lk(list_mu);
      list_snapshots.erase(snap_id);
    }
    if (limit > 0) list_pages.fetch_add(1);
    const bool meta_only = wants_metadata(req);
    std::string out = meta_only ? std::string("{\"apiVersion\":\"meta.k8s.io/v1\",\"kind\":\"PartialObjectMetadataList\"")
                                : "{\"apiVersion\":" + json::quote(p.ti->rt.api_version()) + ",\"kind\":" +
                                      json::quote(p.ti->rt.kind + "List");
    out += ",\"metadata\":{\"resourceVersion\":\"" + rv_str(list_rv) + "\"";
    if (!next.empty()) {
      out += ",\"continue\":" + json::quote(next) +
             ",\"remainingItemCount\":" + std::to_string(items.size() - end);
    }
    out += "},\"items\":[";
    for (size_t i = offset; i < end; ++i) {
      if (i != offset) out.push_back(',');
      if (meta_only) dump_partial_metadata(*items[i], out);
      else items[i]->dump_to(out);
    }
    out += "]}";
    w.send_json(200, out);
  }

  void do_watch(ParsedPath& p, const http::Request& req, http::ResponseWriter& w) {
    auto subp = std::make_shared<WatchSub>();
    WatchSub& sub = *subp;
    sub.type_key = p.ti->key();
    sub.ns = p.ns;
    sub.sel = parse_selector(req.query_param("labelSelector"));
    sub.fields = parse_field_selector(req.query_param("fieldSelector"));
    if (!sub.fields.ns.empty()) sub.ns = sub.fields.ns;
    std::string rv_s = req.query_param("resourceVersion");
    const bool meta_only = wants_metadata(req);
    int timeout_s = opts.max_watch_seconds;
    if (req.has_query_param("timeoutSeconds")) timeout_s = std::min(timeout_s, std::atoi(req.query_param("timeoutSeconds").c_str()));
    bool bookmarks = req.query_param("allowWatchBookmarks") == "true";
    const std::string trace_watch = "kl.watch." + p.ti->rt.plural + "." + field_manager(req, "unknown") + ".sent";
    const std::string trace_written = trace_watch.substr(0, trace_watch.size() - 4) + "written";
    const std::string slow_write = "kw:" + p.ti->rt.plural + " write";
    set_thread_name("kw:" + p.ti->rt.plural);
    struct Rename {
      ~Rename() { set_thread_name("conn:apiserver"); }
    } rename;
    const bool send_initial = req.query_param("sendInitialEvents") == "true";
    if (send_initial && (!bookmarks || req.query_param("resourceVersionMatch") != "NotOlderThan")) {
      throw StatusError(422, "Invalid",
                        "sendInitialEvents requires allowWatchBookmarks=true and resourceVersionMatch=NotOlderThan");
    }
    uint64_t from = 0;
    if (!rv_s.empty() && rv_s != "0" && !parse_rv(rv_s, &from)) {
      throw StatusError(400, "BadRequest", "invalid resource version: " + rv_s);
    }
    std::vector<std::shared_ptr<const std::string>> initial;
    bool gone = false;
    TypeStore& ts = *p.ti->store;
    uint64_t compacted = 0;
    uint64_t initial_rv = 0;
    {
      const bool snapshot = rv_s.empty() || rv_s == "0" || send_initial;
      std::optional<AllShards> shards_lk;
      if (snapshot) shards_lk.emplace(ts, false);
      SharedStoreLock lk(ts.seq, ts.seq_stats);
      compacted = ts.compacted_rv;
      initial_rv = rv.load();
      if (snapshot) {
        for (auto& sh : ts.shards)
        for (auto& [k, st] : sh.objs) {
          const Value& meta = st.obj->get("metadata");
          if (!sub.ns.empty() && meta.get_string("namespace") != sub.ns) continue;
          if (!sub.fields.name_ok(meta.get_string("name"))) continue;
          if (!sub.sel.empty() && !selector_matches(sub.sel, *st.obj)) continue;
          std::string line = "{\"type\":\"ADDED\",\"object\":";
          if (meta_only) dump_partial_metadata(*st.obj, line);
          else st.obj->dump_to(line);
          line += "}\n";
          initial.push_back(std::make_shared<const std::string>(std::move(line)));
        }
      } else if (from < ts.compacted_rv) {
        gone = true;
      } else {
        auto it = std::upper_bound(ts.history.begin(), ts.history.end(), from,
                                   [](uint64_t v, const std::shared_ptr<const EventRec>& e) { return v < e->rv; });
        for (; it != ts.history.end(); ++it) {
          const auto& e = *it;
          if (e->type_key != sub.type_key) continue;
          if (!sub.ns.empty() && e->ns != sub.ns) continue;
          if (!sub.fields.name_ok(e->meta->get("metadata").get_string("name"))) continue;
          View view;
          if (!view_for(sub.sel, *e, &view)) continue;
          if (view == View::AsIs && !meta_only) initial.push_back(e->line);
          else initial.push_back(std::make_shared<const std::string>(e->line_as(view, meta_only)));
        }
      }
      if (!gone) {
        std::lock_guard<std::mutex> wg(ts.watches_mu);
        ts.watches.insert(subp);
      }
    }
    if (!w.start_chunked(200, "application/json")) {
      std::lock_guard<std::mutex> wg(ts.watches_mu);
      ts.watches.erase(subp);
      return;
    }
    if (gone) {
      Value ev = Value::object({{"type", "ERROR"},
                                {"object", status_body(410, "Expired", "too old resource version: " + rv_s + " (" +
                                                                           rv_str(compacted) + ")")}});
      w.write_chunk(ev.dump() + "\n");
      w.end_chunked();
      return;
    }
    bool ok = true;
    for (auto& l : initial) {
      if (!(ok = w.write_chunk(*l))) break;
    }
    if (ok && send_initial) {
      Value bm = Value::object(
          {{"type", "BOOKMARK"},
           {"object", Value::object({{"kind", p.ti->rt.kind},
                                     {"apiVersion", p.ti->rt.api_version()},
                                     {"metadata", Value::object({{"resourceVersion", rv_str(initial_rv)},
                                                                 {"annotations", Value::object({{"k8s.io/initial-events-end", "true"}})}})}})}});
      ok = w.write_chunk(bm.dump() + "\n");
    }
    auto deadline = std::chrono::steady_clock::now() + std::chrono::seconds(timeout_s);
    auto next_bookmark = std::chrono::steady_clock::now() + std::chrono::milliseconds(opts.bookmark_interval_ms);
    while (ok && !w.stopping()) {
      std::vector<QueuedEvent> batch;
      bool closed = false, overflow = false;
      {
        std::unique_lock<std::mutex> lk(sub.m);
        sub.cv.wait_for(lk, std::chrono::milliseconds(500), [&] { return !sub.q.empty() || sub.closed || sub.overflow; });
        const int coalesce_us = watch_coalesce_us.load(std::memory_order_relaxed);
        if (coalesce_us > 0 && !sub.q.empty() && sub.q.size() < 16 && !sub.closed) {
          sub.cv.wait_for(lk, std::chrono::microseconds(coalesce_us),
                          [&] { return sub.q.size() >= 16 || sub.closed || sub.overflow; });
        }
        batch.assign(sub.q.begin(), sub.q.end());
        sub.q.clear();
        closed = sub.closed;
        overflow = sub.overflow;
      }
      if (!batch.empty()) {
        std::string buf;
        for (auto& q : batch) buf += q.e->line_as(q.view, meta_only);
        const bool traced = trace::armed();
        if (traced) {
          for (auto& q : batch) trace::mark(q.e->meta->get("metadata").get_string("name"), trace_watch);
        }
        const int64_t w0 = metrics::now_ns();
        if (!w.write_chunk(buf)) break;
        const int64_t w1 = metrics::now_ns();
        stall::note_slow(slow_write, w0, w1);
        if (traced) {
          for (auto& q : batch) trace::mark_at(q.e->meta->get("metadata").get_string("name"), trace_written, w1);
        }
      }
      if (closed || overflow) break;
      auto now = std::chrono::steady_clock::now();
      if (now >= deadline) break;
      if (bookmarks && now >= next_bookmark) {
        uint64_t cur_rv;
        std::vector<QueuedEvent> pending;
        {
          SharedStoreLock lk(ts.seq, ts.seq_stats);
          cur_rv = rv.load();
          std::lock_guard<std::mutex> g(sub.m);
          pending.assign(sub.q.begin(), sub.q.end());
          sub.q.clear();
        }
        if (!pending.empty()) {
          std::string buf;
          for (auto& q : pending) buf += q.e->line_as(q.view, meta_only);
          if (!w.write_chunk(buf)) break;
        }
        Value bm = Value::object({{"type", "BOOKMARK"},
                                  {"object", Value::object({{"kind", p.ti->rt.kind},
                                                            {"apiVersion", p.ti->rt.api_version()},
                                                            {"metadata", Value::object({{"resourceVersion", rv_str(cur_rv)}})}})}});
        if (!w.write_chunk(bm.dump() + "\n")) break;
        next_bookmark = now + std::chrono::milliseconds(opts.bookmark_interval_ms);
      }
      if (batch.empty() && w.peer_closed()) break;
    }
    {
      std::lock_guard<std::mutex> wg(ts.watches_mu);
      ts.watches.erase(subp);
    }
    w.end_chunked();
  }

  void discovery(const std::string& path, http::ResponseWriter& w) {
    SharedStoreLock lk(types_mu, types_stats);
    if (path == "/api") {
      w.send_json(200, Value::object({{"kind", "APIVersions"}, {"versions", Value::array({"v1"})}}).dump());
      return;
    }
    if (path == "/apis") {
      std::map<std::string, std::set<std::string>> groups;
      for (auto& [k, ti] : types) {
        if (!ti.rt.group.empty()) groups[ti.rt.group].insert(ti.rt.version);
      }
      Value gl = Value::array();
      for (auto& [g, vs] : groups) {
        Value versions = Value::array();
        for (auto& v : vs) versions.push_back(Value::object({{"groupVersion", g + "/" + v}, {"version", v}}));
        gl.push_back(Value::object({{"name", g}, {"versions", versions}, {"preferredVersion", versions[0]}}));
      }
      w.send_json(200, Value::object({{"kind", "APIGroupList"}, {"apiVersion", "v1"}, {"groups", gl}}).dump());
      return;
    }
    std::string gv = path.rfind("/api/", 0) == 0 ? path.substr(5) : path.substr(6);
    Value res = Value::array();
    for (auto& [k, ti] : types) {
      if (ti.rt.api_version() != gv) continue;
      Value verbs = Value::array({"create", "delete", "get", "list", "patch", "update", "watch"});
      res.push_back(Value::object({{"name", ti.rt.plural}, {"namespaced", ti.rt.namespaced}, {"kind", ti.rt.kind}, {"verbs", verbs}}));
      if (ti.rt.has_status) {
        res.push_back(Value::object({{"name", ti.rt.plural + "/status"}, {"namespaced", ti.rt.namespaced}, {"kind", ti.rt.kind},
                                     {"verbs", Value::array({"get", "patch", "update"})}}));
      }
    }
    if (res.empty()) throw StatusError(404, "NotFound", "the server could not find the requested resource");
    w.send_json(200, Value::object({{"kind", "APIResourceList"}, {"apiVersion", "v1"}, {"groupVersion", gv}, {"resources", res}}).dump());
  }

  class HoldingWriter : public http::ResponseWriter {
   public:
    HoldingWriter(http::ResponseWriter& inner, int hold_ms)
        : ResponseWriter(nullptr, inner.keep_alive(), never_stops()), inner_(inner), hold_ms_(hold_ms) {}
    void send(int status, std::string_view body, const std::string& content_type,
              const http::Headers* extra) override {
      inner_.wait_stopping(std::chrono::milliseconds(hold_ms_));
      inner_.send(status, body, content_type, extra);
      sent_ = true;
      status_ = status;
    }
    bool start_chunked(int status, const std::string& content_type) override {
      sent_ = true;
      status_ = status;
      return inner_.start_chunked(status, content_type);
    }
    bool write_chunk(const std::string& data) override { return inner_.write_chunk(data); }
    void end_chunked() override { inner_.end_chunked(); }
    void abort() override { inner_.abort(); }
    bool peer_closed() override { return inner_.peer_closed(); }
    const char* protocol() const override { return inner_.protocol(); }

   private:
    static const CancelToken& never_stops() {
      static const CancelToken t;
      return t;
    }
    http::ResponseWriter& inner_;
    int hold_ms_;
  };

  bool inject_fault(const http::Request& req, http::ResponseWriter& w, int* hold_ms) {
    FaultRule hit;
    bool found = false;
    {
      std::lock_guard<std::mutex> lk(fault_mu);
      for (auto& f : faults) {
        if (f.remaining == 0) continue;
        if (!f.method.empty() && f.method != req.method) continue;
        std::string target = req.path + (req.query.empty() ? "" : "?" + req.query);
        if (!std::regex_search(target, f.path)) continue;
        if (f.remaining > 0) --f.remaining;
        hit = f;
        found = true;
        break;
      }
    }
    if (!found) return false;
    faults_hit.fetch_add(1);
    if (hit.delay_ms > 0 && w.wait_stopping(std::chrono::milliseconds(hit.delay_ms))) {
      w.abort();
      return true;
    }
    if (hit.reset) {
      w.abort();
      return true;
    }
    if (hit.hold_ms > 0 && hit.status <= 0) {
      *hold_ms = hit.hold_ms;
      return false;
    }
    if (hit.status > 0) {
      std::string reason = hit.status == 409   ? "Conflict"
                           : hit.status == 410 ? "Expired"
                           : hit.status == 429 ? "TooManyRequests"
                           : hit.status >= 500 ? "InternalError"
                                               : "BadRequest";
      http::Headers extra;
      if (hit.retry_after_s >= 0) extra.set("Retry-After", std::to_string(hit.retry_after_s));
      w.send(hit.status, status_body(hit.status, reason, hit.message.empty() ? "injected fault" : hit.message).dump(),
             "application/json", &extra);
      return true;
    }
    return false;
  }

  void control(http::Request& req, http::ResponseWriter& w) {
    if (req.path == "/_kl/faults" && req.method == "POST") {
      Value rules = json::parse(req.body);
      std::lock_guard<std::mutex> lk(fault_mu);
      if (req.query_param("append") != "true") faults.clear();
      for (const auto& r : rules.items()) {
        FaultRule f;
        f.method = r.get_string("method");
        f.path_src = r.get_string("path", ".*");
        f.path = std::regex(f.path_src);
        f.status = r.get("status").is_int() ? static_cast<int>(r.get("status").as_int()) : 0;
        f.delay_ms = r.get("delay_ms").is_int() ? static_cast<int>(r.get("delay_ms").as_int()) : 0;
        f.hold_ms = r.get("delay_response_ms").is_int() ? static_cast<int>(r.get("delay_response_ms").as_int()) : 0;
        f.remaining = r.get("count").is_int() ? static_cast<int>(r.get("count").as_int()) : -1;
        f.message = r.get_string("message");
        f.reset = r.get("reset").is_bool() && r.get("reset").as_bool();
        f.retry_after_s = r.get("retry_after").is_int() ? static_cast<int>(r.get("retry_after").as_int()) : -1;
        faults.push_back(std::move(f));
      }
      w.send_json(200, "{}");
      return;
    }
    if (req.path == "/_kl/faults" && req.method == "DELETE") {
      std::lock_guard<std::mutex> lk(fault_mu);
      faults.clear();
      w.send_json(200, "{}");
      return;
    }
    if (req.path == "/_kl/write-latency-us" && req.method == "POST") {
      try {
        size_t used = 0;
        const long long us = std::stoll(req.body, &used);
        if (us < 0 || us > 10000000) throw std::out_of_range("write latency");
        write_latency_us = us;
      } catch (const std::exception&) {
        w.send(400, "body must be 0..10000000 microseconds\n");
        return;
      }
      w.send(200, std::to_string(write_latency_us.load()) + "\n");
      return;
    }
    if (req.path == "/_kl/watch-coalesce-us" && req.method == "POST") {
      int prev = 0;
      try {
        size_t used = 0;
        const long us = std::stol(req.body, &used);
        if (us < 0 || us > 100000) throw std::out_of_range("watch coalesce");
        prev = watch_coalesce_us.exchange(static_cast<int>(us));
      } catch (const std::exception&) {
        w.send(400, "body must be 0..100000 microseconds\n");
        return;
      }
      w.send(200, std::to_string(prev) + "\n");
      return;
    }
    if (req.path == "/_kl/webhook-protocol" && req.method == "POST") {
      const bool h2 = req.body == "h2";
      if (!h2 && req.body != "http/1.1") {
        w.send(400, "body must be h2 or http/1.1\n");
        return;
      }
      {
        std::lock_guard<std::mutex> lk(hook_mu);
        webhook_h2 = h2;
        hook_fast.clear();
        hook_clients.clear();
      }
      w.send(200, h2 ? "h2\n" : "http/1.1\n");
      return;
    }
    if (req.path == "/_kl/compact" && req.method == "POST") {
      uint64_t at = 0;
      for_each_store([&](const std::string&, TypeStore& ts) {
        StoreLock lk(ts.seq, ts.seq_stats);
        at = rv.load();
        ts.compacted_rv = at;
        ts.history.clear();
      });
      w.send_json(200, Value::object({{"compacted_rv", static_cast<unsigned long long>(at)}}).dump());
      return;
    }
    if (req.path == "/_kl/drop-watches" && req.method == "POST") {
      size_t n = 0;
      for_each_store([&](const std::string&, TypeStore& ts) {
        std::lock_guard<std::mutex> wg(ts.watches_mu);
        n += ts.watches.size();
        for (const auto& ws : ts.watches) ws->close();
      });
      w.send_json(200, Value::object({{"dropped", static_cast<unsigned long long>(n)}}).dump());
      return;
    }
    if (req.path == "/_kl/stats") {
      Value counts = Value::object();
      Value locks = Value::object();
      size_t total = 0, n_watches = 0;
      uint64_t acq = 0, contended = 0, wait_ns = 0, hold_ns = 0;
      for_each_store([&](const std::string& key, TypeStore& ts) {
        {
          AllShards lk(ts, false);
          size_t n = 0;
          for (auto& sh : ts.shards) n += sh.objs.size();
          counts[key] = static_cast<unsigned long long>(n);
          total += n;
        }
        {
          std::lock_guard<std::mutex> wg(ts.watches_mu);
          n_watches += ts.watches.size();
        }
        auto account = [](const LockStats& st) {
          return Value::object({{"acquisitions", static_cast<unsigned long long>(st.acquisitions.load())},
                                {"contended", static_cast<unsigned long long>(st.contended.load())},
                                {"wait_ms", static_cast<double>(st.wait_ns.load()) * 1e-6},
                                {"hold_ms", static_cast<double>(st.hold_ns.load()) * 1e-6}});
        };
        for (const LockStats* st : {&ts.stats, &ts.seq_stats}) {
          acq += st->acquisitions.load();
          hold_ns += st->hold_ns.load();
          contended += st->contended.load();
          wait_ns += st->wait_ns.load();
        }
        const uint64_t a = ts.stats.acquisitions.load() + ts.seq_stats.acquisitions.load();
        if (a) {
          locks[key] = Value::object({{"acquisitions", static_cast<unsigned long long>(a)},
                                      {"hold_ms", static_cast<double>(ts.seq_stats.hold_ns.load()) * 1e-6},
                                      {"seq", account(ts.seq_stats)},
                                      {"shards", account(ts.stats)}});
        }
      });
      w.send_json(200, Value::object({{"resourceVersion", static_cast<unsigned long long>(rv.load())},
                                      {"objects", static_cast<unsigned long long>(total)},
                                      {"watches", static_cast<unsigned long long>(n_watches)},
                                      {"requests", static_cast<unsigned long long>(requests.load())},
                                      {"faults_hit", static_cast<unsigned long long>(faults_hit.load())},
                                      {"list_pages", static_cast<unsigned long long>(list_pages.load())},
                                      {"resource_version", rv_str(rv.load())},
                                      {"gc_collected", static_cast<unsigned long long>(gc_collected.load())},
                                      {"store_shards", static_cast<unsigned long long>(opts.store_shards)},
                                      {"gc_pending", static_cast<unsigned long long>([&] {
                                         std::lock_guard<std::mutex> g(gc_mu);
                                         return gc_queue.size();
                                       }())},
                                      {"store_lock", Value::object({
                                          {"acquisitions", static_cast<unsigned long long>(acq)},
                                          {"contended", static_cast<unsigned long long>(contended)},
                                          {"wait_ms", static_cast<double>(wait_ns) * 1e-6},
                                          {"hold_ms", static_cast<double>(hold_ns) * 1e-6}})},
                                      {"by_type_lock", locks},
                                      {"requests_by_kind", [&] {
                                         Value rq = Value::object();
                                         std::lock_guard<std::mutex> g(req_count_mu);
                                         for (auto& [k, v] : req_counts) rq[k] = static_cast<unsigned long long>(v);
                                         return rq;
                                       }()},
                                      {"by_type", counts}}).dump());
      return;
    }
    w.send(404, "not found\n");
  }

  std::mutex req_count_mu;
  std::map<std::string, uint64_t> req_counts;

  void handle(http::Request& req, http::ResponseWriter& w_conn) {
    http::ResponseWriter* wp = &w_conn;
    std::optional<HoldingWriter> holder;
    http::ResponseWriter& w_count = w_conn;
    requests.fetch_add(1, std::memory_order_relaxed);
    std::string res_key = "-";
    struct Count {
      Impl* im;
      const http::Request& req;
      http::ResponseWriter& w;
      std::string& res;
      ~Count() {
        std::string k = req.method + " " + res + " " + std::to_string(w.status_code());
        std::lock_guard<std::mutex> g(im->req_count_mu);
        im->req_counts[k]++;
      }
    } count{this, req, w_count, res_key};
    struct TraceSpan {
      int64_t t_recv = 0;
      ~TraceSpan() {
        if (!t_trace_tag.empty() && !t_trace_name.empty()) {
          trace::mark_at(t_trace_name, t_trace_tag + ".recv", t_recv);
          trace::mark(t_trace_name, t_trace_tag + ".resp");
        }
        t_trace_tag.clear();
        t_trace_name.clear();
      }
    } span;
    if (trace::armed()) span.t_recv = metrics::now_ns();
    try {
      int hold_ms = 0;
      if (inject_fault(req, w_conn, &hold_ms)) return;
      if (hold_ms > 0 && req.method != "GET") wp = &holder.emplace(w_conn, hold_ms);
      http::ResponseWriter& w = *wp;
      UserInfo user = authenticate(req);
      if (req.path == "/apis/authentication.k8s.io/v1/selfsubjectreviews" && req.method == "POST") {
        Value ui = Value::object({{"username", user.username}});
        if (!user.uid.empty()) ui["uid"] = user.uid;
        Value groups = Value::array();
        for (const auto& g : user.groups) groups.push_back(g);
        ui["groups"] = groups;
        w.send_json(201, Value::object({{"kind", "SelfSubjectReview"},
                                        {"apiVersion", "authentication.k8s.io/v1"},
                                        {"metadata", Value::object({{"creationTimestamp", Value()}})},
                                        {"status", Value::object({{"userInfo", ui}})}}).dump());
        return;
      }
      if (req.path == "/api" || req.path == "/apis") {
        discovery(req.path, w);
        return;
      }
      ParsedPath p;
      std::string group, version;
      std::vector<std::string> rest;
      if (!parse_path(req.path, p, group, version, rest)) {
        discovery(req.path, w);
        return;
      }
      res_key = p.ti->rt.plural + (p.sub.empty() ? "" : "/" + p.sub);
      if (p.collection && req.method == "GET") {
        std::string wq = req.query_param("watch");
        if (wq == "1" || wq == "true") res_key += " watch";
      }
      if (span.t_recv && req.method != "GET") {
        t_trace_tag = "kl." + res_key + "." + req.method + "." + field_manager(req, "unknown");
        t_trace_name = p.name;
      }
      if (!p.sub.empty() && p.sub != "status") throw StatusError(404, "NotFound", "subresource not supported: " + p.sub);
      if (!p.sub.empty() && !p.ti->rt.has_status) throw StatusError(404, "NotFound", "the server could not find the requested resource");
      const std::string& m = req.method;
      if (const int64_t lat = write_latency_us.load(std::memory_order_relaxed); lat > 0 && m != "GET") {
        std::this_thread::sleep_for(std::chrono::microseconds(lat));
      }
      if (p.collection) {
        if (m == "GET") {
          std::string wq = req.query_param("watch");
          if (wq == "1" || wq == "true") do_watch(p, req, w);
          else do_list(p, req, w);
        } else if (m == "POST") {
          do_create(p, req, user, w);
        } else {
          throw StatusError(405, "MethodNotAllowed", "method not allowed");
        }
        return;
      }
      if (m == "GET") do_get(p, w, wants_metadata(req));
      else if (m == "PUT") do_update(p, req, user, w);
      else if (m == "PATCH") do_patch(p, req, user, w);
      else if (m == "DELETE") do_delete(p, req, user, w);
      else throw StatusError(405, "MethodNotAllowed", "method not allowed");
    } catch (const StatusError& e) {
      if (!wp->sent()) wp->send_json(e.code, status_body(e.code, e.reason, e.what(), e.details).dump());
    } catch (const std::exception& e) {
      if (!wp->sent()) wp->send_json(500, status_body(500, "InternalError", e.what()).dump());
    }
  }
};

ApiServer::ApiServer(Options o) : impl_(std::make_unique<Impl>(std::move(o))) {}
ApiServer::~ApiServer() { stop(); }

void ApiServer::start() {
  http::ServerOptions so;
  so.addr = impl_->opts.addr;
  so.port = impl_->opts.port;
  so.name = "apiserver";
  so.idle_timeout_ms = 300000;
  if (!impl_->opts.tls_cert_file.empty()) {
    so.tls = net::TlsContext::server_from_files(
        impl_->opts.tls_cert_file, impl_->opts.tls_key_file,
        impl_->opts.client_ca_file.empty() ? "" : net::read_file(impl_->opts.client_ca_file));
  }
  impl_->server = std::make_unique<http::Server>(so);
  Impl* im = impl_.get();
  metrics::set_debug_endpoints(true);
  http::add_standard_routes(*impl_->server);
  impl_->server->handle("GET", "/healthz", [](http::Request&, http::ResponseWriter& w) { w.send(200, "ok"); });
  impl_->server->handle("GET", "/readyz", [](http::Request&, http::ResponseWriter& w) { w.send(200, "ok"); });
  impl_->server->handle("GET", "/livez", [](http::Request&, http::ResponseWriter& w) { w.send(200, "ok"); });
  impl_->server->handle("GET", "/version", [](http::Request&, http::ResponseWriter& w) {
    w.send_json(200, Value::object({{"major", "1"}, {"minor", "26"}, {"gitVersion", "v1.26.0-kube-lite"}, {"platform", "linux/amd64"}}).dump());
  });
  impl_->server->handle_prefix("/api", [im](http::Request& r, http::ResponseWriter& w) { im->handle(r, w); });
  impl_->server->handle_prefix("/_kl/", [im](http::Request& r, http::ResponseWriter& w) { im->control(r, w); });
  impl_->server->start();
}

uint16_t ApiServer::port() const { return impl_->server ? impl_->server->port() : 0; }

void ApiServer::stop() {
  if (impl_ && impl_->server) {
    impl_->for_each_store([](const std::string&, TypeStore& ts) {
      std::lock_guard<std::mutex> wg(ts.watches_mu);
      for (const auto& ws : ts.watches) ws->close();
    });
    impl_->server->stop(std::chrono::milliseconds(2000));
    impl_->server.reset();
  }
}

}
```

native/python/bind_kube.cc:

```cpp
#include <pybind11/pybind11.h>
#include <pybind11/stl.h>

#include <chrono>

#include "apiserver/server.h"
#include "bench/churn.h"
#include "controller/reconcile.h"
#include "kube/events.h"
#include "kube/quantity.h"
#include "kube/ratelimit.h"
#include "kube/runtime.h"

namespace py = pybind11;

namespace bgc_py {

void register_kube(py::module_& m) {
  m.def("desired_children", [](const std::string& ub_json, bool label) {
    std::vector<std::tuple<std::string, std::string, std::string, std::string>> out;
    for (auto& c : bgc::controller::desired_children(bgc::json::parse(ub_json), label))
      out.emplace_back(c.rt->plural, c.ns, c.name, std::move(c.body));
    return out;
  }, py::arg("ub_json"), py::arg("label") = false);
  m.def("quantity_value", [](const std::string& s) -> py::object {
    auto v = bgc::kube::parse_quantity(s);
    return v ? py::object(py::float_(static_cast<double>(*v))) : py::none();
  });
  m.def("same_quantity", [](const std::string& a, const std::string& b) { return bgc::kube::same_quantity(a, b); });
  m.def("canonical_quantity", [](const std::string& s) -> py::object {
    auto c = bgc::kube::canonical_quantity(s);
    return c ? py::object(py::str(*c)) : py::object(py::none());
  });
  py::class_<bgc::bench::ChurnDriver>(m, "ChurnDriver")
      .def(py::init([](const std::string& server, const std::string& token, const std::string& prefix,
                       int concurrency, const std::string& gpu_key, const std::string& group,
                       const std::string& ca_pem, const std::string& approve_url, bool http2,
                       bool server_filter) {
             bgc::bench::ChurnOptions o;
             o.server = server;
             o.admin_token = token;
             o.ca_pem = ca_pem;
             o.name_prefix = prefix;
             o.concurrency = concurrency;
             o.gpu_quota_key = gpu_key;
             o.group = group;
             o.approve_url = approve_url;
             o.http2 = http2;
             o.server_filter = server_filter;
             return std::make_unique<bgc::bench::ChurnDriver>(o);
           }),
           py::arg("server"), py::arg("admin_token"), py::arg("name_prefix"), py::arg("concurrency") = 32,
           py::arg("gpu_quota_key") = "requests.amd.com/gpu", py::arg("group") = "gpu", py::arg("ca_pem") = "",
           py::arg("approve_url") = "", py::arg("http2") = false,
           py::arg("server_filter") = false)
      .def("start", &bgc::bench::ChurnDriver::start)
      .def("step", [](bgc::bench::ChurnDriver& d, const std::vector<std::string>& names, double timeout) {
        bgc::json::Value v;
        {
          py::gil_scoped_release nogil;
          v = d.step(names, timeout);
        }
        return v.dump();
      })
      .def("step_with_delete", [](bgc::bench::ChurnDriver& d, const std::vector<std::string>& names,
                                  const std::vector<std::string>& prev, double timeout) {
        bgc::json::Value v;
        {
          py::gil_scoped_release nogil;
          v = d.step_with_delete(names, prev, timeout);
        }
        return v.dump();
      })
      .def("open_loop", [](bgc::bench::ChurnDriver& d, const std::vector<std::string>& names, double duration_s,
                           double timeout, uint64_t seed) {
        bgc::json::Value v;
        {
          py::gil_scoped_release nogil;
          v = d.open_loop(names, duration_s, timeout, seed);
        }
        return v.dump();
      }, py::arg("names"), py::arg("duration_s"), py::arg("timeout") = 60.0, py::arg("seed") = 1)
      .def("remove", [](bgc::bench::ChurnDriver& d, const std::vector<std::string>& names) {
        py::gil_scoped_release nogil;
        return d.remove(names);
      })
      .def("stop", [](bgc::bench::ChurnDriver& d) {
        py::gil_scoped_release nogil;
        d.stop();
      });

  py::class_<bgc::kube::RetryLimiter>(m, "RetryLimiter")
      .def(py::init([](int64_t base_ms, int64_t cap_ms, double qps, int burst) {
             return std::make_unique<bgc::kube::RetryLimiter>(std::chrono::milliseconds(base_ms),
                                                              std::chrono::milliseconds(cap_ms), qps, burst);
           }),
           py::arg("base_ms") = 5, py::arg("cap_ms") = 60000, py::arg("qps") = 10.0, py::arg("burst") = 100)
      .def("when", [](bgc::kube::RetryLimiter& r, const std::string& k) { return r.when(k).count(); })
      .def("forget", &bgc::kube::RetryLimiter::forget)
      .def("failures", &bgc::kube::RetryLimiter::failures);
  py::class_<bgc::kube::EventRateLimiter>(m, "EventRateLimiter")
      .def(py::init<double, double, size_t>(), py::arg("burst") = 10.0, py::arg("refill_per_minute") = 6.0,
           py::arg("max_keys") = 4096)
      .def("allow", [](bgc::kube::EventRateLimiter& l, const std::string& key, double at_s) {
        return l.allow(key, std::chrono::steady_clock::time_point(
                                std::chrono::duration_cast<std::chrono::steady_clock::duration>(
                                    std::chrono::duration<double>(at_s))));
      })
      .def("size", &bgc::kube::EventRateLimiter::size);
  py::class_<bgc::kube::WorkQueue>(m, "WorkQueue")
      .def(py::init<size_t>(), py::arg("shards") = 1)
      .def("shards", &bgc::kube::WorkQueue::shards)
      .def_static("shards_for", &bgc::kube::WorkQueue::shards_for)
      .def("add", [](bgc::kube::WorkQueue& q, const std::string& k) { q.add(k); })
      .def("add_after", [](bgc::kube::WorkQueue& q, const std::string& k, int ms) { q.add_after(k, std::chrono::milliseconds(ms)); })
      .def("get", [](bgc::kube::WorkQueue& q, size_t worker) {
        std::string k;
        bool ok;
        {
          py::gil_scoped_release nogil;
          ok = q.get(k, worker);
        }
        return ok ? py::object(py::str(k)) : py::object(py::none());
      }, py::arg("worker") = 0)
      .def("done", &bgc::kube::WorkQueue::done)
      .def("forget", &bgc::kube::WorkQueue::forget)
      .def("requeue", [](bgc::kube::WorkQueue& q, const std::string& k, int ms) { q.requeue(k, std::chrono::milliseconds(ms)); })
      .def("shutdown", &bgc::kube::WorkQueue::shutdown)
      .def("pending", &bgc::kube::WorkQueue::pending)
      .def("in_flight", &bgc::kube::WorkQueue::in_flight);
}

}
```

Measured before the change: 10510.

## Rewrite field ownership diffing as single tree walk and avoid managedFields copies

```diff
diff --git a/native/apiserver/fieldset.cc b/native/apiserver/fieldset.cc
--- a/native/apiserver/fieldset.cc
+++ b/native/apiserver/fieldset.cc
@@ -1,6 +1,6 @@
 #include "apiserver/fieldset.h"
 
-#include "core/json_patch.h"
+#include <algorithm>
 
 namespace bgc::apiserver {
 
@@ -8,48 +8,325 @@
 
 namespace {
 
-enum class ListKind { Atomic, KeyedByUid, Set };
-
-ListKind list_kind(const std::string& path) {
-  if (path == "/metadata/ownerReferences") return ListKind::KeyedByUid;
-  if (path == "/metadata/finalizers") return ListKind::Set;
-  return ListKind::Atomic;
-}
-
-bool ignored(const std::string& path, bool include_status) {
-  static const std::set<std::string> kIgnored = {
-      "/apiVersion", "/kind", "/metadata/name", "/metadata/namespace", "/metadata/resourceVersion",
-      "/metadata/uid", "/metadata/generation", "/metadata/creationTimestamp", "/metadata/managedFields",
-      "/metadata/selfLink", "/metadata/deletionTimestamp", "/metadata/deletionGracePeriodSeconds"};
-  if (kIgnored.count(path)) return true;
-  if (!include_status && (path == "/status" || path.rfind("/status/", 0) == 0)) return true;
+enum class Pos : uint8_t { Root, Meta, Owners, Finalizers, Other };
+enum class Status : uint8_t { Skip, Include, Only };
+enum class Kind : uint8_t { Leaf, Object, Keyed };
+
+Pos child_pos(Pos parent, std::string_view key) {
+  if (parent == Pos::Root) return key == "metadata" ? Pos::Meta : Pos::Other;
+  if (parent == Pos::Meta) {
+    if (key == "ownerReferences") return Pos::Owners;
+    if (key == "finalizers") return Pos::Finalizers;
+  }
+  return Pos::Other;
+}
+
+bool ignored_key(Pos parent, std::string_view k, Status st) {
+  if (parent == Pos::Root) {
+    if (k == "status") return st == Status::Skip;
+    return st == Status::Only || k == "apiVersion" || k == "kind";
+  }
+  if (parent != Pos::Meta) return false;
+  return k == "name" || k == "namespace" || k == "resourceVersion" || k == "uid" || k == "generation" ||
+         k == "creationTimestamp" || k == "managedFields" || k == "selfLink" || k == "deletionTimestamp" ||
+         k == "deletionGracePeriodSeconds";
+}
+
+Kind kind_of(const Value& v, Pos pos) {
+  if (v.is_object() && !v.empty()) return Kind::Object;
+  if (v.is_array() && !v.empty() && (pos == Pos::Owners || pos == Pos::Finalizers)) return Kind::Keyed;
+  return Kind::Leaf;
+}
+
+bool is_item_token(std::string_view t) { return t.size() >= 3 && t.front() == '[' && t.back() == ']'; }
+
+struct Path {
+  std::string s;
+  void escaped(std::string_view t) {
+    for (char c : t) {
+      if (c == '~') s += "~0";
+      else if (c == '/') s += "~1";
+      else s.push_back(c);
+    }
+  }
+  size_t key(std::string_view k) {
+    const size_t n = s.size();
+    s.push_back('/');
+    escaped(k);
+    return n;
+  }
+  size_t owner(std::string_view uid) {
+    const size_t n = s.size();
+    s += "/[uid=";
+    escaped(uid);
+    s.push_back(']');
+    return n;
+  }
+  size_t member(std::string_view dumped) {
+    const size_t n = s.size();
+    s += "/[=";
+    escaped(dumped);
+    s.push_back(']');
+    return n;
+  }
+  void cut(size_t n) { s.resize(n); }
+};
+
+std::string_view token_uid(const Value& item) {
+  const Value* u = item.find("uid");
+  return u && u->is_string() ? std::string_view(u->as_string()) : std::string_view();
+}
+const Value* first_owner(const Value& list, std::string_view uid) {
+  for (const auto& item : list.items()) {
+    const Value* u = item.find("uid");
+    if (u && u->is_string() && u->as_string() == uid) return &item;
+  }
+  return nullptr;
+}
+bool has_token_uid(const Value& list, std::string_view uid) {
+  for (const auto& item : list.items()) {
+    if (token_uid(item) == uid) return true;
+  }
   return false;
 }
-
-void collect(const Value& v, const std::string& path, FieldSet& out, bool include_status) {
-  if (!path.empty() && ignored(path, include_status)) return;
-  if (v.is_object() && !v.empty()) {
-    const auto& keys = v.keys();
-    const auto& vals = v.values();
-    for (size_t i = 0; i < keys.size(); ++i) {
-      collect(vals[i], path + "/" + json::escape_pointer_token(keys[i]), out, include_status);
-    }
-    return;
-  }
-  if (v.is_array() && !v.empty()) {
-    ListKind lk = list_kind(path);
-    if (lk == ListKind::KeyedByUid) {
+const Value* first_equal(const Value& list, const Value& want) {
+  for (const auto& item : list.items()) {
+    if (item == want) return &item;
+  }
+  return nullptr;
+}
+
+template <class F>
+void walk(const Value& v, Pos pos, Status st, Path& p, F& f) {
+  switch (kind_of(v, pos)) {
+    case Kind::Object: {
+      const auto& keys = v.keys();
+      const auto& vals = v.values();
+      for (size_t i = 0; i < keys.size(); ++i) {
+        if (ignored_key(pos, keys[i], st)) continue;
+        const size_t n = p.key(keys[i]);
+        walk(vals[i], child_pos(pos, keys[i]), st, p, f);
+        p.cut(n);
+      }
+      return;
+    }
+    case Kind::Keyed:
       for (const auto& item : v.items()) {
-        out.insert(path + "/[uid=" + json::escape_pointer_token(item.get_string("uid")) + "]");
-      }
-      return;
-    }
-    if (lk == ListKind::Set) {
-      for (const auto& item : v.items()) out.insert(path + "/[=" + json::escape_pointer_token(item.dump()) + "]");
-      return;
-    }
-  }
-  if (!path.empty()) out.insert(path);
+        const size_t n = pos == Pos::Owners ? p.owner(token_uid(item)) : p.member(item.dump());
+        f(p.s, item);
+        p.cut(n);
+      }
+      return;
+    case Kind::Leaf:
+      if (pos != Pos::Root) f(p.s, v);
+  }
+}
+
+struct Diff {
+  Status st;
+  Path p;
+  FieldSet& changed;
+  FieldSet& removed;
+
+  void all_changed(const Value& a, Pos pos) {
+    auto f = [&](const std::string& path, const Value&) { changed.insert(path); };
+    walk(a, pos, st, p, f);
+  }
+  void all_removed(const Value& b, Pos pos) {
+    auto f = [&](const std::string& path, const Value&) { removed.insert(path); };
+    walk(b, pos, st, p, f);
+  }
+  void disjoint(const Value& b, const Value& a, Pos pos) {
+    FieldSet in_a;
+    auto fa = [&](const std::string& path, const Value&) { in_a.insert(path); };
+    walk(a, pos, st, p, fa);
+    auto fb = [&](const std::string& path, const Value&) {
+      if (!in_a.count(path)) removed.insert(path);
+    };
+    walk(b, pos, st, p, fb);
+    changed.merge(in_a);
+  }
+
+  void node(const Value* b, const Value* a, Pos pos, bool readable) {
+    if (pos == Pos::Root && b && kind_of(*b, pos) == Kind::Leaf) b = nullptr;
+    if (pos == Pos::Root && a && kind_of(*a, pos) == Kind::Leaf) a = nullptr;
+    if (!a) {
+      if (b) all_removed(*b, pos);
+      return;
+    }
+    if (!b) return all_changed(*a, pos);
+    const Kind kind = kind_of(*a, pos);
+    if (!readable || kind != kind_of(*b, pos)) return disjoint(*b, *a, pos);
+    if (kind == Kind::Leaf) {
+      if (!(*b == *a)) changed.insert(p.s);
+      return;
+    }
+    if (kind == Kind::Object) {
+      const auto& keys = a->keys();
+      const auto& vals = a->values();
+      for (size_t i = 0; i < keys.size(); ++i) {
+        if (ignored_key(pos, keys[i], st)) continue;
+        const size_t n = p.key(keys[i]);
+        node(b->find(keys[i]), &vals[i], child_pos(pos, keys[i]), !is_item_token(keys[i]));
+        p.cut(n);
+      }
+      const auto& bkeys = b->keys();
+      for (size_t i = 0; i < bkeys.size(); ++i) {
+        if (ignored_key(pos, bkeys[i], st) || a->contains(bkeys[i])) continue;
+        const size_t n = p.key(bkeys[i]);
+        all_removed(b->values()[i], child_pos(pos, bkeys[i]));
+        p.cut(n);
+      }
+      return;
+    }
+    if (pos == Pos::Owners) {
+      for (const auto& item : a->items()) {
+        const std::string_view uid = token_uid(item);
+        const Value* av = first_owner(*a, uid);
+        const Value* bv = first_owner(*b, uid);
+        if (av && bv && *av == *bv) continue;
+        const size_t n = p.owner(uid);
+        changed.insert(p.s);
+        p.cut(n);
+      }
+      for (const auto& item : b->items()) {
+        const std::string_view uid = token_uid(item);
+        if (has_token_uid(*a, uid)) continue;
+        const size_t n = p.owner(uid);
+        removed.insert(p.s);
+        p.cut(n);
+      }
+      return;
+    }
+    std::vector<std::string> in_a, in_b;
+    for (const auto& item : a->items()) in_a.push_back(item.dump());
+    for (const auto& item : b->items()) in_b.push_back(item.dump());
+    for (const auto& d : in_a) {
+      if (std::find(in_b.begin(), in_b.end(), d) != in_b.end()) continue;
+      const size_t n = p.member(d);
+      changed.insert(p.s);
+      p.cut(n);
+    }
+    for (const auto& d : in_b) {
+      if (std::find(in_a.begin(), in_a.end(), d) != in_a.end()) continue;
+      const size_t n = p.member(d);
+      removed.insert(p.s);
+      p.cut(n);
+    }
+  }
+};
+
+struct Applied {
+  Status st;
+  Path p;
+  std::vector<AppliedLeaf>& out;
+
+  void leaf(const Value* want, const Value* have, bool readable) {
+    out.push_back({p.s, readable ? want : nullptr, readable ? have : nullptr});
+  }
+  void node(const Value& cfg, const Value* have, Pos pos, bool readable) {
+    switch (kind_of(cfg, pos)) {
+      case Kind::Object: {
+        const auto& keys = cfg.keys();
+        const auto& vals = cfg.values();
+        for (size_t i = 0; i < keys.size(); ++i) {
+          if (ignored_key(pos, keys[i], st)) continue;
+          const size_t n = p.key(keys[i]);
+          node(vals[i], have ? have->find(keys[i]) : nullptr, child_pos(pos, keys[i]),
+               readable && !is_item_token(keys[i]));
+          p.cut(n);
+        }
+        return;
+      }
+      case Kind::Keyed: {
+        const Value* list = have && have->is_array() ? have : nullptr;
+        for (const auto& item : cfg.items()) {
+          if (pos == Pos::Owners) {
+            const std::string_view uid = token_uid(item);
+            const size_t n = p.owner(uid);
+            leaf(first_owner(cfg, uid), list ? first_owner(*list, uid) : nullptr, readable);
+            p.cut(n);
+          } else {
+            const size_t n = p.member(item.dump());
+            leaf(first_equal(cfg, item), list ? first_equal(*list, item) : nullptr, readable);
+            p.cut(n);
+          }
+        }
+        return;
+      }
+      case Kind::Leaf:
+        if (pos != Pos::Root) leaf(&cfg, have, readable);
+    }
+  }
+};
+
+bool writes_any(const Value& cfg, Pos pos, Status st) {
+  switch (kind_of(cfg, pos)) {
+    case Kind::Object: {
+      const auto& keys = cfg.keys();
+      for (size_t i = 0; i < keys.size(); ++i) {
+        if (ignored_key(pos, keys[i], st) || is_item_token(keys[i])) continue;
+        if (writes_any(cfg.values()[i], child_pos(pos, keys[i]), st)) return true;
+      }
+      return false;
+    }
+    case Kind::Keyed:
+      if (pos == Pos::Finalizers) return true;
+      for (const auto& item : cfg.items()) {
+        const Value* u = item.find("uid");
+        if (u && u->is_string()) return true;
+      }
+      return false;
+    case Kind::Leaf:
+      return pos != Pos::Root;
+  }
+  return false;
+}
+
+void merge(Value& live, const Value& cfg, Pos pos, Status st) {
+  switch (kind_of(cfg, pos)) {
+    case Kind::Object: {
+      if (!live.is_object()) live = Value::object();
+      const auto& keys = cfg.keys();
+      const auto& vals = cfg.values();
+      for (size_t i = 0; i < keys.size(); ++i) {
+        if (ignored_key(pos, keys[i], st) || is_item_token(keys[i])) continue;
+        const Pos cp = child_pos(pos, keys[i]);
+        if (writes_any(vals[i], cp, st)) merge(live[keys[i]], vals[i], cp, st);
+      }
+      return;
+    }
+    case Kind::Keyed: {
+      if (!live.is_array()) live = Value::array();
+      std::vector<std::pair<std::string, const Value*>> items;
+      Path token;
+      for (const auto& item : cfg.items()) {
+        if (pos == Pos::Owners) {
+          const std::string_view uid = token_uid(item);
+          const Value* want = first_owner(cfg, uid);
+          if (!want) continue;
+          token.cut(0);
+          token.owner(uid);
+          items.emplace_back(token.s, want);
+        } else {
+          token.cut(0);
+          token.member(item.dump());
+          items.emplace_back(token.s, first_equal(cfg, item));
+        }
+      }
+      std::sort(items.begin(), items.end(), [](const auto& x, const auto& y) { return x.first < y.first; });
+      items.erase(std::unique(items.begin(), items.end(), [](const auto& x, const auto& y) { return x.first == y.first; }),
+                  items.end());
+      for (const auto& [tok, want] : items) {
+        const Value* at = pos == Pos::Owners ? first_owner(live, token_uid(*want)) : first_equal(live, *want);
+        if (at) live[static_cast<size_t>(at - live.items().data())] = *want;
+        else live.push_back(*want);
+      }
+      return;
+    }
+    case Kind::Leaf:
+      if (pos != Pos::Root) live = cfg;
+  }
 }
 
 class Tokens {
@@ -86,8 +363,6 @@
   std::string scratch_;
 };
 
-bool is_item_token(std::string_view t) { return t.size() >= 3 && t.front() == '[' && t.back() == ']'; }
-
 long find_item(const Value& arr, std::string_view tok) {
   std::string_view inner = tok.substr(1, tok.size() - 2);
   if (inner.substr(0, 4) == "uid=") {
@@ -112,26 +387,10 @@
 
 FieldSet leaves(const Value& obj, bool include_status) {
   FieldSet fs;
-  collect(obj, "", fs, include_status);
+  Path p;
+  auto f = [&](const std::string& path, const Value&) { fs.insert(path); };
+  walk(obj, Pos::Root, include_status ? Status::Include : Status::Skip, p, f);
   return fs;
-}
-
-const Value* get_path(const Value& root, const std::string& path) {
-  const Value* cur = &root;
-  Tokens ts(path);
-  std::string_view t;
-  while (ts.next(t)) {
-    if (is_item_token(t)) {
-      if (!cur->is_array()) return nullptr;
-      long i = find_item(*cur, t);
-      if (i < 0) return nullptr;
-      cur = &(*cur)[static_cast<size_t>(i)];
-    } else {
-      cur = cur->find(t);
-      if (!cur) return nullptr;
-    }
-  }
-  return cur;
 }
 
 bool remove_path(Value& root, const std::string& path) {
@@ -158,60 +417,32 @@
   return false;
 }
 
-void set_path(Value& root, const std::string& path, const Value& v) {
-  Value* cur = &root;
-  Tokens ts(path);
-  std::string_view t;
-  while (ts.next(t)) {
-    const bool last = ts.last();
-    if (is_item_token(t)) {
-      if (!cur->is_array()) *cur = Value::array();
-      long i = find_item(*cur, t);
-      if (i < 0) {
-        cur->push_back(last ? v : Value::object());
-        cur = &(*cur)[cur->size() - 1];
-      } else {
-        cur = &(*cur)[static_cast<size_t>(i)];
-        if (last) *cur = v;
-      }
-      continue;
-    }
-    if (!cur->is_object()) *cur = Value::object();
-    if (last) {
-      (*cur)[t] = v;
-    } else {
-      cur = &(*cur)[t];
-    }
-  }
-}
-
 void diff_leaves(const Value& before, const Value& after, FieldSet& changed, FieldSet& removed, bool include_status) {
-  FieldSet b = leaves(before, include_status);
-  FieldSet a = leaves(after, include_status);
-  for (const auto& p : a) {
-    const Value* bv = b.count(p) ? get_path(before, p) : nullptr;
-    const Value* av = get_path(after, p);
-    if (!bv || !av || !(*bv == *av)) changed.insert(p);
-  }
-  for (const auto& p : b) {
-    if (!a.count(p)) removed.insert(p);
-  }
+  Diff d{include_status ? Status::Include : Status::Skip, {}, changed, removed};
+  d.node(&before, &after, Pos::Root, true);
 }
 
 void diff_member_leaves(const Value& before, const Value& after, const std::string& key, FieldSet& changed,
                         FieldSet& removed) {
-  const std::string base = "/" + json::escape_pointer_token(key);
-  FieldSet b, a;
-  if (const Value* v = before.find(key)) collect(*v, base, b, true);
-  if (const Value* v = after.find(key)) collect(*v, base, a, true);
-  for (const auto& p : a) {
-    const Value* bv = b.count(p) ? get_path(before, p) : nullptr;
-    const Value* av = get_path(after, p);
-    if (!bv || !av || !(*bv == *av)) changed.insert(p);
-  }
-  for (const auto& p : b) {
-    if (!a.count(p)) removed.insert(p);
-  }
+  if (ignored_key(Pos::Root, key, Status::Include)) return;
+  Diff d{Status::Include, {}, changed, removed};
+  d.p.key(key);
+  d.node(before.find(key), after.find(key), child_pos(Pos::Root, key), !is_item_token(key));
+}
+
+std::vector<AppliedLeaf> applied_leaves(const Value& config, const Value& live, bool status_only) {
+  std::vector<AppliedLeaf> out;
+  Applied a{status_only ? Status::Only : Status::Skip, {}, out};
+  a.node(config, &live, Pos::Root, true);
+  std::sort(out.begin(), out.end(), [](const AppliedLeaf& x, const AppliedLeaf& y) { return x.path < y.path; });
+  out.erase(std::unique(out.begin(), out.end(), [](const AppliedLeaf& x, const AppliedLeaf& y) { return x.path == y.path; }),
+            out.end());
+  return out;
+}
+
+void merge_applied(Value& live, const Value& config, bool status_only) {
+  const Status st = status_only ? Status::Only : Status::Skip;
+  if (writes_any(config, Pos::Root, st)) merge(live, config, Pos::Root, st);
 }
 
 std::string display_path(const std::string& path) {
diff --git a/native/apiserver/fieldset.h b/native/apiserver/fieldset.h
--- a/native/apiserver/fieldset.h
+++ b/native/apiserver/fieldset.h
@@ -1,6 +1,5 @@
 #pragma once
 
-#include <map>
 #include <set>
 #include <string>
 #include <vector>
@@ -12,13 +11,20 @@
 using FieldSet = std::set<std::string>;
 
 FieldSet leaves(const json::Value& obj, bool include_status = false);
-const json::Value* get_path(const json::Value& root, const std::string& path);
 bool remove_path(json::Value& root, const std::string& path);
-void set_path(json::Value& root, const std::string& path, const json::Value& v);
 void diff_leaves(const json::Value& before, const json::Value& after, FieldSet& changed, FieldSet& removed,
                  bool include_status = false);
 void diff_member_leaves(const json::Value& before, const json::Value& after, const std::string& key,
                         FieldSet& changed, FieldSet& removed);
+
+struct AppliedLeaf {
+  std::string path;
+  const json::Value* want;
+  const json::Value* have;
+};
+std::vector<AppliedLeaf> applied_leaves(const json::Value& config, const json::Value& live, bool status_only);
+void merge_applied(json::Value& live, const json::Value& config, bool status_only);
+
 std::string display_path(const std::string& path);
 json::Value fields_v1(const FieldSet& fs);
 
diff --git a/native/apiserver/server.cc b/native/apiserver/server.cc
--- a/native/apiserver/server.cc
+++ b/native/apiserver/server.cc
@@ -253,11 +253,47 @@
   std::string time;
   std::string subresource;
   FieldSet fields;
+  Value rendered;
   bool operator==(const ManagerEntry& o) const {
     return operation == o.operation && fields == o.fields && subresource == o.subresource;
   }
 };
-using Managers = std::map<std::string, ManagerEntry>;
+using Managers = std::map<std::string, std::shared_ptr<const ManagerEntry>>;
+
+std::shared_ptr<const ManagerEntry> seal(const std::string& key, ManagerEntry e) {
+  e.rendered = Value::object({{"manager", key.substr(0, key.find('\x1f'))}, {"operation", e.operation},
+                              {"apiVersion", e.api_version}, {"time", e.time}, {"fieldsType", "FieldsV1"},
+                              {"fieldsV1", fields_v1(e.fields)}});
+  if (!e.subresource.empty()) e.rendered["subresource"] = e.subresource;
+  return std::make_shared<const ManagerEntry>(std::move(e));
+}
+
+bool same_managers(const Managers& a, const Managers& b) {
+  if (a.size() != b.size()) return false;
+  for (auto ia = a.begin(), ib = b.begin(); ia != a.end(); ++ia, ++ib) {
+    if (ia->first != ib->first) return false;
+    if (ia->second != ib->second && !(*ia->second == *ib->second)) return false;
+  }
+  return true;
+}
+
+Value copy_without_managed(const Value& obj) {
+  const Value* meta = obj.find("metadata");
+  if (!meta || !meta->is_object() || !meta->contains("managedFields")) return obj;
+  Value out = Value::object();
+  for (size_t i = 0; i < obj.keys().size(); ++i) {
+    const std::string& k = obj.keys()[i];
+    if (k != "metadata") {
+      out[k] = obj.values()[i];
+      continue;
+    }
+    Value& m = out[k] = Value::object();
+    for (size_t j = 0; j < meta->keys().size(); ++j) {
+      if (meta->keys()[j] != "managedFields") m[meta->keys()[j]] = meta->values()[j];
+    }
+  }
+  return out;
+}
 
 inline const std::shared_ptr<const Managers>& no_managers() {
   static const std::shared_ptr<const Managers> empty = std::make_shared<const Managers>();
@@ -1060,8 +1096,43 @@
     return c;
   }
 
+  static void dump_with_managed(const Value& obj, const Value* managed, std::string& out) {
+    const Value* meta = obj.find("metadata");
+    if (!managed || !meta || !meta->is_object() || meta->contains("managedFields")) return obj.dump_to(out);
+    out += '{';
+    for (size_t i = 0; i < obj.keys().size(); ++i) {
+      if (i) out += ',';
+      out += json::quote(obj.keys()[i]);
+      out += ':';
+      if (&obj.values()[i] != meta) {
+        obj.values()[i].dump_to(out);
+        continue;
+      }
+      out += '{';
+      for (size_t j = 0; j < meta->keys().size(); ++j) {
+        out += json::quote(meta->keys()[j]);
+        out += ':';
+        meta->values()[j].dump_to(out);
+        out += ',';
+      }
+      out += "\"managedFields\":";
+      managed->dump_to(out);
+      out += '}';
+    }
+    out += '}';
+  }
+
+  static bool append_committed_object(const std::string* line, std::string& out) {
+    static const std::string kObjectKey = ",\"object\":";
+    const size_t at = line ? line->find(kObjectKey) : std::string::npos;
+    if (at == std::string::npos || line->size() < at + kObjectKey.size() + 2) return false;
+    out.append(*line, at + kObjectKey.size(), line->size() - (at + kObjectKey.size()) - 2);
+    return true;
+  }
+
   void call_webhooks(const TypeInfo& ti, const std::string& sub, const std::string& op, const std::string& ns,
-                     const std::string& name, Value* obj, const Value* old, const UserInfo& user) {
+                     const std::string& name, Value* obj, const Value* old, const UserInfo& user,
+                     const Value* managed = nullptr, const std::string* old_line = nullptr) {
     auto hooks = matching_webhooks(ti, sub, op);
     if (hooks.empty()) return;
     static auto& hist = metrics::Registry::global().histogram("kl_webhook_duration_seconds", "Webhook callout latency");
@@ -1095,11 +1166,11 @@
       body += ",\"userInfo\":";
       user.to_json().dump_to(body);
       body += ",\"object\":";
-      if (obj) obj->dump_to(body);
+      if (obj) dump_with_managed(*obj, managed, body);
       else body += "null";
       body += ",\"oldObject\":";
-      if (old) old->dump_to(body);
-      else body += "null";
+      if (!old) body += "null";
+      else if (!append_committed_object(old_line, body)) old->dump_to(body);
       body += ",\"dryRun\":false,\"options\":{\"kind\":" + json::quote(opts_kind) +
               ",\"apiVersion\":\"meta.k8s.io/v1\"}}}";
       std::string err;
@@ -1251,7 +1322,7 @@
   static bool is_core_namespaces(const TypeInfo& ti) { return ti.rt.plural == "namespaces" && ti.rt.group.empty(); }
 
   std::shared_ptr<const Value> terminate_namespace_locked(const TypeInfo& ti, const std::string& name, Stored& cur) {
-    Value obj = *cur.obj;
+    Value obj = copy_without_managed(*cur.obj);
     obj["metadata"]["deletionTimestamp"] = now_rfc3339();
     obj["metadata"]["deletionGracePeriodSeconds"] = 0;
     obj["status"]["phase"] = "Terminating";
@@ -1274,22 +1345,16 @@
       erase_locked(*nti, "", name);
       return;
     }
-    Value obj = *it->second.obj;
+    Value obj = copy_without_managed(*it->second.obj);
     if (obj.get("spec").get("finalizers").empty()) return;
     obj["spec"]["finalizers"] = Value::array();
     commit_locked(*nti, "", name, std::move(obj), *it->second.managers, &it->second);
   }
 
-  static void render_managed(Value& obj, const Managers& m, const std::string& api_version) {
+  static void render_managed(Value& obj, const Managers& m) {
     Value arr = Value::array();
     for (const auto& [key, e] : m) {
-      if (e.fields.empty()) continue;
-      std::string mgr = key.substr(0, key.find('\x1f'));
-      Value ent = Value::object({{"manager", mgr}, {"operation", e.operation},
-                                 {"apiVersion", e.api_version.empty() ? api_version : e.api_version},
-                                 {"time", e.time}, {"fieldsType", "FieldsV1"}, {"fieldsV1", fields_v1(e.fields)}});
-      if (!e.subresource.empty()) ent["subresource"] = e.subresource;
-      arr.push_back(std::move(ent));
+      if (!e->fields.empty()) arr.push_back(e->rendered);
     }
     if (arr.empty()) obj["metadata"].erase("managedFields");
     else obj["metadata"]["managedFields"] = std::move(arr);
@@ -1348,26 +1413,42 @@
     FieldSet changed, removed;
     if (status_write) diff_member_leaves(before, after, "status", changed, removed);
     else diff_leaves(before, after, changed, removed);
-    for (auto& [name, e] : m) {
-      for (const auto& p : changed) e.fields.erase(p);
+    const std::string writer = status_write ? manager + "\x1fstatus" : manager;
+    auto owns_any = [](const FieldSet& fields, const FieldSet& paths) {
+      return std::any_of(paths.begin(), paths.end(), [&](const std::string& p) { return fields.count(p) > 0; });
+    };
+    for (auto it = m.begin(); it != m.end();) {
+      const ManagerEntry& cur = *it->second;
+      const bool writes = !changed.empty() && it->first == writer;
+      if (!writes && !owns_any(cur.fields, changed) && !owns_any(cur.fields, removed)) {
+        ++it;
+        continue;
+      }
+      ManagerEntry e{cur.operation, cur.api_version, cur.time, cur.subresource, cur.fields, Value()};
       for (const auto& p : removed) e.fields.erase(p);
-    }
-    if (!changed.empty()) {
-      auto& e = m[status_write ? manager + "\x1fstatus" : manager];
-      if (e.operation.empty()) {
+      if (writes) {
         e.operation = "Update";
-        e.api_version = api_version;
-      }
-      if (e.operation == "Apply") {
-        e.operation = "Update";
-      }
+        e.time = now_rfc3339();
+        if (status_write) e.subresource = "status";
+        e.fields.insert(changed.begin(), changed.end());
+      } else {
+        for (const auto& p : changed) e.fields.erase(p);
+      }
+      if (e.fields.empty()) {
+        it = m.erase(it);
+      } else {
+        it->second = seal(it->first, std::move(e));
+        ++it;
+      }
+    }
+    if (!changed.empty() && !m.count(writer)) {
+      ManagerEntry e;
+      e.operation = "Update";
+      e.api_version = api_version;
       e.time = now_rfc3339();
       if (status_write) e.subresource = "status";
-      for (const auto& p : changed) e.fields.insert(p);
-    }
-    for (auto it = m.begin(); it != m.end();) {
-      if (it->second.fields.empty()) it = m.erase(it);
-      else ++it;
+      e.fields = std::move(changed);
+      m[writer] = seal(writer, std::move(e));
     }
   }
 
@@ -1375,10 +1456,9 @@
     static const std::string p = "\x01rv\x01";
     return p;
   }
-  static PreparedEvent prepare_commit(Value& obj, const Managers& managers, const std::string& api_version,
-                                      const char* type) {
+  static PreparedEvent prepare_commit(Value& obj, const Managers& managers, const char* type) {
     obj["metadata"]["resourceVersion"] = rv_placeholder();
-    render_managed(obj, managers, api_version);
+    render_managed(obj, managers);
     std::string line = std::string("{\"type\":\"") + type + "\",\"object\":";
     obj.dump_to(line);
     line += "}\n";
@@ -1402,7 +1482,7 @@
     TypeStore& ts = *ti.store;
     PreparedEvent local;
     if (!pe || !pe->ok) {
-      local = prepare_commit(obj, managers, ti.rt.api_version(), prev ? "MODIFIED" : "ADDED");
+      local = prepare_commit(obj, managers, prev ? "MODIFIED" : "ADDED");
       pe = &local;
     }
     std::string key = obj_key(ti.rt, ns, name);
@@ -1486,15 +1566,8 @@
     std::shared_ptr<const Value> ptr = it->second.obj;
     std::string line = "{\"type\":\"DELETED\",\"object\":";
     const size_t obj_at = line.size();
-    static const std::string kObjectKey = ",\"object\":";
     const std::shared_ptr<const std::string> held = it->second.line.lock();
-    const std::string* committed = held.get();
-    const size_t at = committed ? committed->find(kObjectKey) : std::string::npos;
-    if (at != std::string::npos && committed->size() >= at + kObjectKey.size() + 2) {
-      line.append(*committed, at + kObjectKey.size(), committed->size() - (at + kObjectKey.size()) - 2);
-    } else {
-      ptr->dump_to(line);
-    }
+    if (!append_committed_object(held.get(), line)) ptr->dump_to(line);
     line += "}\n";
     const std::string old_rv = "\"resourceVersion\":" + json::quote(ptr->get("metadata").get_string("resourceVersion"));
     const size_t pos = line.find(old_rv, obj_at);
@@ -1615,7 +1688,12 @@
     }
   }
 
-  using Compute = std::function<std::pair<Value, Managers>(const Stored* cur)>;
+  struct Computed {
+    Value obj;
+    Managers managers;
+    bool managed_left_out = false;
+  };
+  using Compute = std::function<Computed(const Stored* cur)>;
 
   WriteResult write(TypeInfo& ti, const std::string& ns, const std::string& name, const std::string& sub,
                     const UserInfo& user, const Compute& compute, bool allow_create, bool is_status) {
@@ -1633,7 +1711,9 @@
         }
       }
       if (!exists && !allow_create) throw not_found(ti.rt, name);
-      auto [obj, managers] = compute(exists ? &cur_copy : nullptr);
+      Computed computed = compute(exists ? &cur_copy : nullptr);
+      Value& obj = computed.obj;
+      Managers& managers = computed.managers;
       canonicalize_quantities(ti, obj);
       std::string op = exists ? "UPDATE" : "CREATE";
       if (!exists && ti.rt.namespaced) {
@@ -1653,18 +1733,23 @@
                                                                      {"field", "metadata.namespace"}})})}}));
         }
       }
-      if (exists && same_content(obj, *cur_copy.obj) && managers == *cur_copy.managers) {
+      if (exists && same_content(obj, *cur_copy.obj) && same_managers(managers, *cur_copy.managers)) {
         return {cur_copy.obj, 200, nullptr};
       }
       trace_step(name, ".hook0");
-      call_webhooks(ti, sub, op, ns, name, &obj, exists ? cur_copy.obj.get() : nullptr, user);
+      {
+        const std::shared_ptr<const std::string> stored_line = cur_copy.line.lock();
+        call_webhooks(ti, sub, op, ns, name, &obj, exists ? cur_copy.obj.get() : nullptr, user,
+                      exists && computed.managed_left_out ? cur_copy.obj->get("metadata").find("managedFields") : nullptr,
+                      stored_line.get());
+      }
       trace_step(name, ".hook1");
       obj["metadata"]["name"] = name;
       if (ti.rt.namespaced) obj["metadata"]["namespace"] = ns;
       else obj["metadata"].erase("namespace");
       canonicalize_quantities(ti, obj);
       validate_object(ti, name, ns, obj);
-      if (exists && same_content(obj, *cur_copy.obj) && managers == *cur_copy.managers) {
+      if (exists && same_content(obj, *cur_copy.obj) && same_managers(managers, *cur_copy.managers)) {
         return {cur_copy.obj, 200, nullptr};
       }
       if (exists && spec_changed(*cur_copy.obj, obj)) {
@@ -1673,7 +1758,7 @@
                           : 1;
         obj["metadata"]["generation"] = gen + 1;
       }
-      PreparedEvent pe = prepare_commit(obj, managers, ti.rt.api_version(), exists ? "MODIFIED" : "ADDED");
+      PreparedEvent pe = prepare_commit(obj, managers, exists ? "MODIFIED" : "ADDED");
       StoreLock lk(sh.mu, ti.store->stats);
       auto it = sh.objs.find(key);
       bool now_exists = it != sh.objs.end();
@@ -1773,13 +1858,13 @@
     std::string manager = field_manager(req, "unknown");
     if (!t_trace_tag.empty()) t_trace_name = name;
     auto res = write(*p.ti, p.ns, name, "", user,
-                     [&](const Stored* cur) -> std::pair<Value, Managers> {
+                     [&](const Stored* cur) -> Computed {
                        if (cur) throw already_exists(p.ti->rt, name);
                        Value obj = body;
                        init_new(*p.ti, obj, p.ns, name);
                        Managers m;
                        attribute_update(m, manager, Value::object(), obj, false, p.ti->rt.api_version());
-                       return {std::move(obj), std::move(m)};
+                       return {std::move(obj), std::move(m), false};
                      },
                      true, false);
     {
@@ -1800,14 +1885,14 @@
     bool is_status = p.sub == "status";
     std::string manager = field_manager(req, "unknown");
     auto res = write(*p.ti, p.ns, p.name, p.sub, user,
-                     [&](const Stored* cur) -> std::pair<Value, Managers> {
+                     [&](const Stored* cur) -> Computed {
                        std::string want_rv = body.get("metadata").get_string("resourceVersion");
                        if (!want_rv.empty() && want_rv != cur->obj->get("metadata").get_string("resourceVersion")) {
                          throw conflict(p.ti->rt, p.name);
                        }
                        Value obj;
                        if (is_status) {
-                         obj = *cur->obj;
+                         obj = copy_without_managed(*cur->obj);
                          if (body.contains("status")) obj["status"] = body.get("status");
                          else obj.erase("status");
                        } else {
@@ -1820,7 +1905,7 @@
                        }
                        Managers m = *cur->managers;
                        attribute_update(m, manager, *cur->obj, obj, is_status, p.ti->rt.api_version());
-                       return {std::move(obj), std::move(m)};
+                       return {std::move(obj), std::move(m), is_status};
                      },
                      false, is_status);
     {
@@ -1830,35 +1915,25 @@
     }
   }
 
-  std::pair<Value, Managers> apply_ssa(const TypeInfo& ti, const Stored* cur, const Value& config,
-                                       const std::string& manager_name, bool force, bool is_status,
-                                       const std::string& ns, const std::string& name) {
+  Computed apply_ssa(const TypeInfo& ti, const Stored* cur, const Value& config, const std::string& manager_name,
+                     bool force, bool is_status, const std::string& ns, const std::string& name) {
     const std::string manager = is_status ? manager_name + "\x1fstatus" : manager_name;
-    FieldSet cfg_fields = leaves(config, is_status);
-    if (is_status) {
-      FieldSet only;
-      for (const auto& f : cfg_fields) {
-        if (f == "/status" || f.rfind("/status/", 0) == 0) only.insert(f);
-      }
-      cfg_fields.swap(only);
-    }
-    Value live;
+    Value fresh;
+    if (!cur) {
+      fresh = Value::object();
+      init_new(ti, fresh, ns, name);
+    }
+    std::vector<AppliedLeaf> cfg = applied_leaves(config, cur ? *cur->obj : fresh, is_status);
     Managers m;
-    if (cur) {
-      live = *cur->obj;
-      m = *cur->managers;
-    } else {
-      live = Value::object();
-      init_new(ti, live, ns, name);
-    }
-    std::vector<std::pair<std::string, std::string>> conflicts;
-    for (const auto& f : cfg_fields) {
-      const Value* want = get_path(config, f);
-      const Value* have = get_path(live, f);
-      for (auto& [other, e] : m) {
-        if (other == manager || !e.fields.count(f)) continue;
-        if (have && want && *have == *want) continue;
-        conflicts.emplace_back(other, f);
+    if (cur) m = *cur->managers;
+    std::vector<std::pair<const std::string*, const std::string*>> conflicts;
+    const bool others = m.size() > 1 || (m.size() == 1 && m.begin()->first != manager);
+    for (size_t i = 0; others && i < cfg.size(); ++i) {
+      const AppliedLeaf& l = cfg[i];
+      for (const auto& [other, e] : m) {
+        if (other == manager || !e->fields.count(l.path)) continue;
+        if (l.have && l.want && *l.have == *l.want) continue;
+        conflicts.emplace_back(&other, &l.path);
       }
     }
     if (!conflicts.empty() && !force) {
@@ -1866,41 +1941,57 @@
                         (conflicts.size() > 1 ? "s" : "") + ": ";
       for (size_t i = 0; i < conflicts.size(); ++i) {
         if (i) msg += "; ";
-        msg += "conflict with \"" + conflicts[i].first.substr(0, conflicts[i].first.find('\x1f')) + "\": " +
-               display_path(conflicts[i].second);
+        msg += "conflict with \"" + conflicts[i].first->substr(0, conflicts[i].first->find('\x1f')) + "\": " +
+               display_path(*conflicts[i].second);
       }
       throw StatusError(409, "Conflict", msg);
     }
-    if (force) {
-      for (const auto& [other, f] : conflicts) m[other].fields.erase(f);
-    }
+    if (!conflicts.empty()) {
+      std::map<std::string, ManagerEntry> losing;
+      for (const auto& [other, f] : conflicts) {
+        auto it = losing.find(*other);
+        if (it == losing.end()) {
+          const ManagerEntry& e = *m.at(*other);
+          it = losing.emplace(*other, ManagerEntry{e.operation, e.api_version, e.time, e.subresource, e.fields, Value()}).first;
+        }
+        it->second.fields.erase(*f);
+      }
+      for (auto& [other, e] : losing) {
+        if (e.fields.empty()) m.erase(other);
+        else m[other] = seal(other, std::move(e));
+      }
+    }
+    FieldSet fields;
+    for (auto& l : cfg) fields.emplace_hint(fields.end(), std::move(l.path));
+    cfg.clear();
+    Value live = cur ? copy_without_managed(*cur->obj) : std::move(fresh);
     if (auto it = m.find(manager); it != m.end()) {
-      for (const auto& f : it->second.fields) {
-        if (cfg_fields.count(f)) continue;
+      for (const auto& f : it->second->fields) {
+        if (fields.count(f)) continue;
         bool other_owner = false;
-        for (auto& [other, e] : m) {
-          if (other != manager && e.fields.count(f)) other_owner = true;
+        for (const auto& [other, e] : m) {
+          if (other != manager && e->fields.count(f)) other_owner = true;
         }
         if (!other_owner) remove_path(live, f);
       }
     }
-    for (const auto& f : cfg_fields) {
-      if (const Value* v = get_path(config, f)) set_path(live, f, *v);
-    }
-    auto& me = m[manager];
-    me.operation = "Apply";
-    me.api_version = ti.rt.api_version();
-    me.time = now_rfc3339();
-    me.subresource = is_status ? "status" : "";
-    me.fields = cfg_fields;
-    for (auto it = m.begin(); it != m.end();) {
-      if (it->second.fields.empty()) it = m.erase(it);
-      else ++it;
+    merge_applied(live, config, is_status);
+    if (fields.empty()) {
+      m.erase(manager);
+    } else {
+      ManagerEntry me;
+      me.operation = "Apply";
+      me.api_version = ti.rt.api_version();
+      me.time = now_rfc3339();
+      me.subresource = is_status ? "status" : "";
+      me.fields = std::move(fields);
+      m[manager] = seal(manager, std::move(me));
     }
     if (cur && ti.rt.has_status && !is_status) {
-      if (cur->obj->contains("status")) live["status"] = cur->obj->get("status");
-    }
-    return {std::move(live), std::move(m)};
+      const Value* status = cur->obj->find("status");
+      if (status && !(live.get("status") == *status)) live["status"] = *status;
+    }
+    return {std::move(live), std::move(m), cur != nullptr};
   }
 
   void do_patch(ParsedPath& p, const http::Request& req, const UserInfo& user, http::ResponseWriter& w) {
@@ -1914,7 +2005,7 @@
     Value patch = parse_body(req);
     bool force = req.query_param("force") == "true";
     auto res = write(*p.ti, p.ns, p.name, p.sub, user,
-                     [&](const Stored* cur) -> std::pair<Value, Managers> {
+                     [&](const Stored* cur) -> Computed {
                        if (is_apply) {
                          std::string pname = patch.get("metadata").get_string("name");
                          if (!pname.empty() && pname != p.name) {
@@ -1923,9 +2014,11 @@
                          }
                          return apply_ssa(*p.ti, cur, patch, manager, force, is_status, p.ns, p.name);
                        }
-                       Value obj = *cur->obj;
+                       const bool json_patch = ct.find("json-patch") != std::string::npos;
+                       const bool full = json_patch || patch.get("metadata").contains("managedFields");
+                       Value obj = full ? *cur->obj : copy_without_managed(*cur->obj);
                        try {
-                         if (ct.find("json-patch") != std::string::npos) {
+                         if (json_patch) {
                            json::apply_patch(obj, patch);
                          } else {
                            json::apply_merge_patch(obj, patch);
@@ -1938,7 +2031,7 @@
                          throw conflict(p.ti->rt, p.name);
                        }
                        if (is_status) {
-                         Value keep = *cur->obj;
+                         Value keep = copy_without_managed(*cur->obj);
                          if (obj.contains("status")) keep["status"] = obj.get("status");
                          else keep.erase("status");
                          obj = std::move(keep);
@@ -1951,7 +2044,7 @@
                        }
                        Managers m = *cur->managers;
                        attribute_update(m, manager, *cur->obj, obj, is_status, p.ti->rt.api_version());
-                       return {std::move(obj), std::move(m)};
+                       return {std::move(obj), std::move(m), is_status || !full};
                      },
                      is_apply, is_status);
     {
@@ -1986,7 +2079,7 @@
     }
     if (!meta.get("finalizers").empty()) {
       if (!meta.contains("deletionTimestamp")) {
-        Value obj = *it->second.obj;
+        Value obj = copy_without_managed(*it->second.obj);
         obj["metadata"]["deletionTimestamp"] = now_rfc3339();
         obj["metadata"]["deletionGracePeriodSeconds"] = 0;
         auto ptr = commit_locked(*p.ti, p.ns, p.name, std::move(obj), *it->second.managers, &it->second);
diff --git a/native/python/bind_kube.cc b/native/python/bind_kube.cc
--- a/native/python/bind_kube.cc
+++ b/native/python/bind_kube.cc
@@ -3,6 +3,7 @@
 
 #include <chrono>
 
+#include "apiserver/fieldset.h"
 #include "apiserver/server.h"
 #include "bench/churn.h"
 #include "controller/reconcile.h"
@@ -31,6 +32,45 @@
     auto c = bgc::kube::canonical_quantity(s);
     return c ? py::object(py::str(*c)) : py::object(py::none());
   });
+  auto paths_json = [](const bgc::apiserver::FieldSet& fs) {
+    bgc::json::Value a = bgc::json::Value::array();
+    for (const auto& p : fs) a.push_back(p);
+    return a;
+  };
+  m.def("fieldset_leaves", [paths_json](const std::string& obj, bool include_status) {
+    return paths_json(bgc::apiserver::leaves(bgc::json::parse(obj), include_status)).dump();
+  }, py::arg("obj"), py::arg("include_status") = false);
+  m.def("fieldset_diff", [paths_json](const std::string& before, const std::string& after, bool include_status) {
+    bgc::apiserver::FieldSet changed, removed;
+    bgc::apiserver::diff_leaves(bgc::json::parse(before), bgc::json::parse(after), changed, removed, include_status);
+    return bgc::json::Value::object({{"changed", paths_json(changed)}, {"removed", paths_json(removed)}}).dump();
+  }, py::arg("before"), py::arg("after"), py::arg("include_status") = false);
+  m.def("fieldset_diff_member", [paths_json](const std::string& before, const std::string& after,
+                                             const std::string& key) {
+    bgc::apiserver::FieldSet changed, removed;
+    bgc::apiserver::diff_member_leaves(bgc::json::parse(before), bgc::json::parse(after), key, changed, removed);
+    return bgc::json::Value::object({{"changed", paths_json(changed)}, {"removed", paths_json(removed)}}).dump();
+  });
+  m.def("fieldset_apply", [](const std::string& config, const std::string& live, bool status_only) {
+    const bgc::json::Value cfg = bgc::json::parse(config);
+    bgc::json::Value obj = bgc::json::parse(live);
+    bgc::json::Value rows = bgc::json::Value::array();
+    for (const auto& l : bgc::apiserver::applied_leaves(cfg, obj, status_only)) {
+      bgc::json::Value row = bgc::json::Value::object({{"path", l.path}});
+      if (l.want) row["want"] = *l.want;
+      if (l.have) row["have"] = *l.have;
+      rows.push_back(std::move(row));
+    }
+    bgc::apiserver::merge_applied(obj, cfg, status_only);
+    return bgc::json::Value::object({{"leaves", std::move(rows)}, {"merged", std::move(obj)}}).dump();
+  });
+  m.def("fieldset_fields_v1",[](const std::string& paths) {
+    bgc::apiserver::FieldSet fs;
+    const bgc::json::Value list = bgc::json::parse(paths);
+    for (const auto& p : list.items()) fs.insert(p.as_string());
+    return bgc::apiserver::fields_v1(fs).dump();
+  });
+  m.def("fieldset_display_path", [](const std::string& path) { return bgc::apiserver::display_path(path); });
   py::class_<bgc::bench::ChurnDriver>(m, "ChurnDriver")
       .def(py::init([](const std::string& server, const std::string& token, const std::string& prefix,
                        int concurrency, const std::string& gpu_key, const std::string& group,
diff --git a/profiles/kl_write_path/shares.py b/profiles/kl_write_path/shares.py
--- /dev/null
+++ b/profiles/kl_write_path/shares.py
@@ -0,0 +1,43 @@
+#!/usr/bin/env python3
+import re
+import sys
+
+OWNERSHIP = re.compile(r"::(leaves|get_path|set_path|remove_path|diff_leaves|diff_member_leaves|fields_v1|applied_leaves|"
+                       r"merge_applied|seal|same_managers|copy_without_managed|collect|walk|merge|writes_any)[<(]|"
+                       r"::(Diff|Applied|Path)::|attribute_update|render_managed|apply_ssa")
+ALLOC = re.compile(r"(^|;)(malloc|free|cfree|__default_morecore|operator new|operator delete|__nss_database_lookup)[^;]*$")
+ROWS = [
+    ("write() inclusive", lambda s: "Impl::write" in s),
+    ("do_patch inclusive", lambda s: "Impl::do_patch" in s),
+    ("prepare_commit inclusive", lambda s: "prepare_commit" in s),
+    ("allocator (leaf frames)", lambda s: ALLOC.search(s) is not None),
+    ("field ownership", lambda s: OWNERSHIP.search(s) is not None or ("Impl::write" in s and "_Rb_tree" in s)),
+    ("  with compute and prepare_commit", lambda s: OWNERSHIP.search(s) is not None or (
+        "Impl::write" in s and ("_Rb_tree" in s or "prepare_commit" in s or "_Function_handler" in s))),
+    ("now_rfc3339", lambda s: "now_rfc3339" in s or "rfc3339_micro_now" in s),
+    ("call_webhooks: serialization", lambda s: re.search(r"call_webhooks[^;]*;[^;]*(dump_impl|dump_to|dump_with_managed)", s) is not None),
+]
+
+
+def main(path):
+    total = attributed = 0
+    counts = {name: [0, 0] for name, _ in ROWS}
+    for line in open(path):
+        stack, n = line.rsplit(" ", 1)
+        n = int(n)
+        rooted = "_M_run" in stack
+        total += n
+        attributed += n if rooted else 0
+        for name, hit in ROWS:
+            if hit(stack):
+                counts[name][0] += n
+                counts[name][1] += n if rooted else 0
+    print(f"samples {total}, attributed {attributed} ({100.0 * attributed / total:.1f} %)")
+    print(f"{'':36s}{'% of all':>10s}{'% of attributed':>18s}")
+    for name, _ in ROWS:
+        a, r = counts[name]
+        print(f"{name:36s}{100.0 * a / total:10.2f}{100.0 * r / attributed:18.2f}")
+
+
+if __name__ == "__main__":
+    main(sys.argv[1])
```

Result: slower. 9561 (-9.1%).
